# PrimeIntellect-ai/OpenDiloco

Measured on AMD Instinct MI355X. Metric: tokens_per_second, higher is better.
Workload: dtype bf16; 1 GPU; llama-150m DiLoCo, 1 worker(s), H=50, bf16, total-batch 512/worker, seq 1024 (BASELINE.json configs[1]); model=llama-150m, global_batch=512, seq_len=1024, parallelism=diloco-dp1, grad_acc=8, per_device_batch=64, params=214983680

## Files before the change

opendiloco_amd/csrc/attn.hip:

```cpp

#include "dk_common.h"
#include "../../include/diloco_kernels.h"

#include <math.h>
#include <stdlib.h>

typedef __attribute__((ext_vector_type(8))) _Float16 halfx8;

template <int DT> struct MFMA16;
template <> struct MFMA16<2> {
  using frag = shortx8;
  static __device__ __forceinline__ floatx4 mma(frag a, frag b, floatx4 c) {
    return __builtin_amdgcn_mfma_f32_16x16x32_bf16(a, b, c, 0, 0, 0);
  }
};
template <> struct MFMA16<1> {
  using frag = halfx8;
  static __device__ __forceinline__ floatx4 mma(frag a, frag b, floatx4 c) {
    return __builtin_amdgcn_mfma_f32_16x16x32_f16(a, b, c, 0, 0, 0);
  }
};

template <int DT> struct TrRead;
template <> struct TrRead<2> {
  typedef __attribute__((ext_vector_type(4))) __bf16 v4;
  static __device__ __forceinline__ void rd(const unsigned short* p, void* out) {
    v4 r = __builtin_amdgcn_ds_read_tr16_b64_v4bf16(
        (__attribute__((address_space(3))) v4*)(uintptr_t)(const void*)p);
    __builtin_memcpy(out, &r, 8);
  }
};
template <> struct TrRead<1> {
  typedef __attribute__((ext_vector_type(4))) __fp16 v4;
  static __device__ __forceinline__ void rd(const _Float16* p, void* out) {
    v4 r = __builtin_amdgcn_ds_read_tr16_b64_v4f16(
        (__attribute__((address_space(3))) v4*)(uintptr_t)(const void*)p);
    __builtin_memcpy(out, &r, 8);
  }
};
template <int DT>
__device__ __forceinline__ typename MFMA16<DT>::frag trread_bfrag(
    const typename DTraits<DT>::T* img, int row0, int col0, int ds, int lane) {
  const int rb = row0 + 8 * (lane >> 4) + ((lane & 15) >> 2);
  const int cb = col0 + 4 * (lane & 3);
  typename MFMA16<DT>::frag f;
  TrRead<DT>::rd(img + rb * ds + cb, &f);
  TrRead<DT>::rd(img + (rb + 4) * ds + cb, (char*)&f + 8);
  return f;
}

template <int DT> struct Pack4;
template <> struct Pack4<2> { using V = shortx4; };
template <> struct Pack4<1> { typedef __attribute__((ext_vector_type(4))) _Float16 V; };

#define NEG_BIG (-1e30f)

__device__ __forceinline__ float grp16_max(float x) {
#pragma unroll
  for (int off = 1; off < 16; off <<= 1) x = fmaxf(x, __shfl_xor(x, off, DK_WAVE));
  return x;
}
__device__ __forceinline__ float grp16_sum(float x) {
#pragma unroll
  for (int off = 1; off < 16; off <<= 1) x += __shfl_xor(x, off, DK_WAVE);
  return x;
}


template <int DT, int D>
__global__ __launch_bounds__(256) void attn_fwd_kernel(
    typename DTraits<DT>::T* __restrict__ o, float* __restrict__ lse,
    const typename DTraits<DT>::T* __restrict__ q,
    const typename DTraits<DT>::T* __restrict__ k,
    const typename DTraits<DT>::T* __restrict__ v,
    int B, int Hq, int Hkv, int S, float scale,
    int64_t o_sb, int64_t o_sh, int64_t o_sr,
    int64_t v_sb, int64_t v_sh, int64_t v_sr) {
  using TR = DTraits<DT>;
  using T = typename TR::T;
  using MF = MFMA16<DT>;
  using frag = typename MF::frag;
  constexpr int KT = 64;
  constexpr int KS = KT + 8;
  constexpr int DS = D + 8;
  constexpr int NKC = D / 32;
  constexpr int NDN = D / 16;
  constexpr int NNT = KT / 16;
  constexpr int LPT = (KT * D) / 8 / 256;

  extern __shared__ __attribute__((aligned(16))) char smem_raw[];
  T* K_lds = (T*)smem_raw;
  T* V_lds = K_lds + 2 * KT * DS;
  T* P_lds = V_lds + 2 * KT * DS;

  const int lane = threadIdx.x & 63;
  const int wave = threadIdx.x >> 6;
  const int lo = lane & 15;
  const int hi = lane >> 4;

  const int nQT = (S + 63) / 64;
  int bid = blockIdx.x;
  const int qt = bid % nQT;
  const int h = (bid / nQT) % Hq;
  const int b = bid / (nQT * Hq);
  const int hkv = h / (Hq / Hkv);

  const int q0 = qt * 64 + wave * 16;
  const int64_t qoff = (((int64_t)b * Hq + h) * S) * D;
  const int64_t kvoff = (((int64_t)b * Hkv + hkv) * S) * D;
  const int64_t voff = v_sb ? ((int64_t)b * v_sb + (int64_t)hkv * v_sh) : kvoff;
  const int64_t v_rs = v_sb ? v_sr : (int64_t)D;

  frag q_frag[NKC];
  {
    const int qrow = q0 + lo;
    const int qr_c = qrow < S ? qrow : S - 1;
#pragma unroll
    for (int kc = 0; kc < NKC; ++kc)
      q_frag[kc] = *(const frag*)(q + qoff + (int64_t)qr_c * D + kc * 32 + hi * 8);
  }

  float m_run[4], l_run[4];
  floatx4 o_acc[NDN];
#pragma unroll
  for (int r = 0; r < 4; ++r) { m_run[r] = NEG_BIG; l_run[r] = 0.f; }
#pragma unroll
  for (int dn = 0; dn < NDN; ++dn) o_acc[dn] = (floatx4)(0.f);

  const int kv_end = min(S, qt * 64 + 64);
  const int n_kt = (kv_end + KT - 1) / KT;

  frag kreg[LPT], vreg[LPT];
  const int st_row[2] = {(int)threadIdx.x / (D / 8), (int)(threadIdx.x + 256) / (D / 8)};
  const int st_c8[2] = {((int)threadIdx.x % (D / 8)) * 8, ((int)(threadIdx.x + 256) % (D / 8)) * 8};

  auto load_tile = [&](int kt) {
#pragma unroll
    for (int i = 0; i < LPT; ++i) {
      const int krow = kt * KT + st_row[i];
      const int kr_c = krow < S ? krow : S - 1;
      kreg[i] = *(const frag*)(k + kvoff + (int64_t)kr_c * D + st_c8[i]);
      vreg[i] = *(const frag*)(v + voff + (int64_t)kr_c * v_rs + st_c8[i]);
    }
  };
  auto write_tile = [&](int buf) {
    T* Kb = K_lds + buf * KT * DS;
    T* Vb = V_lds + buf * KT * DS;
#pragma unroll
    for (int i = 0; i < LPT; ++i) {
      *(frag*)(Kb + st_row[i] * DS + st_c8[i]) = kreg[i];
      *(frag*)(Vb + st_row[i] * DS + st_c8[i]) = vreg[i];
    }
  };

  load_tile(0);
  write_tile(0);
  __syncthreads();

  for (int kt = 0; kt < n_kt; ++kt) {
    const int kbase = kt * KT;
    const int cur = kt & 1;
    T* Kb = K_lds + cur * KT * DS;
    T* Vb = V_lds + cur * KT * DS;
    if (kt + 1 < n_kt) load_tile(kt + 1);

    floatx4 sc[NNT];
    __builtin_amdgcn_s_setprio(1);
#pragma unroll
    for (int nt = 0; nt < NNT; ++nt) {
      sc[nt] = (floatx4)(0.f);
#pragma unroll
      for (int kc = 0; kc < NKC; ++kc) {
        frag bk = *(const frag*)(Kb + (nt * 16 + lo) * DS + kc * 32 + hi * 8);
        sc[nt] = MF::mma(q_frag[kc], bk, sc[nt]);
      }
    }
    __builtin_amdgcn_s_setprio(0);

    const bool full_tile = (kbase + KT <= q0) && (kbase + KT <= S);
    float p[NNT][4];
#pragma unroll
    for (int r = 0; r < 4; ++r) {
      const int qrow = q0 + hi * 4 + r;
      float rm = NEG_BIG;
      float sv[NNT];
      if (full_tile) {
#pragma unroll
        for (int nt = 0; nt < NNT; ++nt) {
          sv[nt] = sc[nt][r] * scale;
          rm = fmaxf(rm, sv[nt]);
        }
      } else {
#pragma unroll
        for (int nt = 0; nt < NNT; ++nt) {
          const int kk = kbase + nt * 16 + lo;
          sv[nt] = (kk > qrow || kk >= S) ? NEG_BIG : sc[nt][r] * scale;
          rm = fmaxf(rm, sv[nt]);
        }
      }
      rm = grp16_max(rm);
      const float m_new = fmaxf(m_run[r], rm);
      const float alpha = __expf(m_run[r] - m_new);
      float psum = 0.f;
#pragma unroll
      for (int nt = 0; nt < NNT; ++nt) {
        p[nt][r] = sv[nt] <= NEG_BIG ? 0.f : __expf(sv[nt] - m_new);
        psum += p[nt][r];
      }
      l_run[r] = l_run[r] * alpha + grp16_sum(psum);
      m_run[r] = m_new;
#pragma unroll
      for (int dn = 0; dn < NDN; ++dn) o_acc[dn][r] *= alpha;
    }

    T* Pw = P_lds + wave * 16 * KS;
#pragma unroll
    for (int nt = 0; nt < NNT; ++nt)
#pragma unroll
      for (int r = 0; r < 4; ++r) Pw[(hi * 4 + r) * KS + nt * 16 + lo] = TR::fromF(p[nt][r]);
    frag pa[KT / 32];
#pragma unroll
    for (int c = 0; c < KT / 32; ++c)
      pa[c] = *(const frag*)(Pw + lo * KS + c * 32 + hi * 8);

    __builtin_amdgcn_s_setprio(1);
#pragma unroll
    for (int dn = 0; dn < NDN; ++dn)
#pragma unroll
      for (int c = 0; c < KT / 32; ++c) {
        frag bv = trread_bfrag<DT>(Vb, c * 32, dn * 16, DS, lane);
        o_acc[dn] = MF::mma(pa[c], bv, o_acc[dn]);
      }
    __builtin_amdgcn_s_setprio(0);

    if (kt + 1 < n_kt) write_tile((kt + 1) & 1);
    __syncthreads();
  }

#pragma unroll
  for (int r = 0; r < 4; ++r) {
    const int qrow = q0 + hi * 4 + r;
    if (qrow >= S) continue;
    const float inv_l = l_run[r] > 0.f ? 1.f / l_run[r] : 0.f;
    const int64_t obase = (int64_t)b * o_sb + (int64_t)h * o_sh + (int64_t)qrow * o_sr;
#pragma unroll
    for (int dn = 0; dn < NDN; ++dn)
      o[obase + dn * 16 + lo] = TR::fromF(o_acc[dn][r] * inv_l);
    if (lo == 0) lse[((int64_t)b * Hq + h) * S + qrow] = m_run[r] + __logf(l_run[r]);
  }
}

typedef __attribute__((ext_vector_type(16))) float floatx16;
typedef __attribute__((ext_vector_type(4))) int intx4;

template <int DT> struct MFMA32;
template <> struct MFMA32<2> {
  using frag = shortx8;
  static __device__ __forceinline__ floatx16 mma(frag a, frag b, floatx16 c) {
    return __builtin_amdgcn_mfma_f32_32x32x16_bf16(a, b, c, 0, 0, 0);
  }
};
template <> struct MFMA32<1> {
  using frag = halfx8;
  static __device__ __forceinline__ floatx16 mma(frag a, frag b, floatx16 c) {
    return __builtin_amdgcn_mfma_f32_32x32x16_f16(a, b, c, 0, 0, 0);
  }
};

template <int DT>
__device__ __forceinline__ typename MFMA32<DT>::frag trread_afrag32(
    const typename DTraits<DT>::T* img, int row0, int col0, int ds, int lane) {
  const int lam = lane & 15;
  const int rb = row0 + 8 * (lane >> 5) + (lam >> 2);
  const int cb = col0 + 16 * ((lane >> 4) & 1) + 4 * (lam & 3);
  typename MFMA32<DT>::frag f;
  TrRead<DT>::rd(img + rb * ds + cb, &f);
  TrRead<DT>::rd(img + (rb + 4) * ds + cb, (char*)&f + 8);
  return f;
}

template <int DT, int D>
__global__ __launch_bounds__(256, 4) void attn_fwd_v3_kernel(
    typename DTraits<DT>::T* __restrict__ o, float* __restrict__ lse,
    const typename DTraits<DT>::T* __restrict__ q,
    const typename DTraits<DT>::T* __restrict__ k,
    const typename DTraits<DT>::T* __restrict__ v,
    int B, int Hq, int Hkv, int S, float scale,
    int64_t o_sb, int64_t o_sh, int64_t o_sr,
    int64_t v_sb, int64_t v_sh, int64_t v_sr) {
  using TR = DTraits<DT>;
  using T = typename TR::T;
  using MF = MFMA32<DT>;
  using frag = typename MF::frag;
  constexpr int KT = 64;
  constexpr int KS = KT + 8;
  constexpr int DS = D + 8;
  constexpr int NKC = D / 16;
  constexpr int NMT = D / 32;
  constexpr int LPT = (KT * D) / 8 / 256;

  extern __shared__ __attribute__((aligned(16))) char smem_raw[];
  T* K_lds = (T*)smem_raw;
  T* V_lds = K_lds + 2 * KT * DS;

  const int lane = threadIdx.x & 63;
  const int wave = threadIdx.x >> 6;
  const int lo32 = lane & 31;
  const int hi5 = lane >> 5;

  const int nQT = (S + 127) / 128;
  int bid = blockIdx.x;
  const int qt = bid % nQT;
  const int h = (bid / nQT) % Hq;
  const int b = bid / (nQT * Hq);
  const int hkv = h / (Hq / Hkv);

  const int q0 = qt * 128 + wave * 32;
  const int qrow = q0 + lo32;
  const int64_t qoff = (((int64_t)b * Hq + h) * S) * D;
  const int64_t kvoff = (((int64_t)b * Hkv + hkv) * S) * D;
  const int64_t voff = v_sb ? ((int64_t)b * v_sb + (int64_t)hkv * v_sh) : kvoff;
  const int64_t v_rs = v_sb ? v_sr : (int64_t)D;

  frag q_frag[NKC];
  {
    const int qr_c = qrow < S ? qrow : S - 1;
#pragma unroll
    for (int kc = 0; kc < NKC; ++kc)
      q_frag[kc] = *(const frag*)(q + qoff + (int64_t)qr_c * D + kc * 16 + hi5 * 8);
  }

  float m_run = NEG_BIG, l_run = 0.f;
  floatx16 oacc[NMT];
#pragma unroll
  for (int mt = 0; mt < NMT; ++mt) oacc[mt] = (floatx16)(0.f);

  const int kv_end = min(S, qt * 128 + 128);
  const int n_kt = (kv_end + KT - 1) / KT;

  shortx8 kreg[LPT], vreg[LPT];
  const int st_row[2] = {(int)threadIdx.x / (D / 8), (int)(threadIdx.x + 256) / (D / 8)};
  const int st_c8[2] = {((int)threadIdx.x % (D / 8)) * 8, ((int)(threadIdx.x + 256) % (D / 8)) * 8};

  auto load_tile = [&](int kt) {
#pragma unroll
    for (int i = 0; i < LPT; ++i) {
      const int krow = kt * KT + st_row[i];
      const int kr_c = krow < S ? krow : S - 1;
      kreg[i] = *(const shortx8*)(k + kvoff + (int64_t)kr_c * D + st_c8[i]);
      vreg[i] = *(const shortx8*)(v + voff + (int64_t)kr_c * v_rs + st_c8[i]);
    }
  };
  auto write_tile = [&](int buf) {
    T* Kb = K_lds + buf * KT * DS;
    T* Vb = V_lds + buf * KT * DS;
#pragma unroll
    for (int i = 0; i < LPT; ++i) {
      *(shortx8*)(Kb + st_row[i] * DS + st_c8[i]) = kreg[i];
      *(shortx8*)(Vb + st_row[i] * DS + st_c8[i]) = vreg[i];
    }
  };

  load_tile(0);
  write_tile(0);
  __syncthreads();

  for (int kt = 0; kt < n_kt; ++kt) {
    const int kbase = kt * KT;
    const int cur = kt & 1;
    T* Kb = K_lds + cur * KT * DS;
    T* Vb = V_lds + cur * KT * DS;
    if (kt + 1 < n_kt) load_tile(kt + 1);

#pragma unroll
    for (int st = 0; st < 2; ++st) {
      const int sbase = kbase + st * 32;
      if (sbase >= q0 + 32) continue;
      floatx16 sc = (floatx16)(0.f);
      __builtin_amdgcn_s_setprio(1);
#pragma unroll
      for (int kc = 0; kc < NKC; ++kc) {
        frag ka = *(const frag*)(Kb + (st * 32 + lo32) * DS + kc * 16 + hi5 * 8);
        sc = MF::mma(ka, q_frag[kc], sc);
      }
      __builtin_amdgcn_s_setprio(0);

      const bool full_tile = (sbase + 32 <= q0) && (sbase + 32 <= S);
      float rm = NEG_BIG;
      if (full_tile) {
#pragma unroll
        for (int r = 0; r < 16; ++r) {
          sc[r] *= scale;
          rm = fmaxf(rm, sc[r]);
        }
      } else {
#pragma unroll
        for (int r = 0; r < 16; ++r) {
          const int key = sbase + (r & 3) + 8 * (r >> 2) + 4 * hi5;
          sc[r] = (key > qrow || key >= S) ? NEG_BIG : sc[r] * scale;
          rm = fmaxf(rm, sc[r]);
        }
      }
      rm = fmaxf(rm, __shfl_xor(rm, 32, DK_WAVE));
      const float m_new = fmaxf(m_run, rm);
      const float alpha = __expf(m_run - m_new);
      float psum = 0.f;
#pragma unroll
      for (int r = 0; r < 16; ++r) {
        sc[r] = sc[r] <= NEG_BIG ? 0.f : __expf(sc[r] - m_new);
        psum += sc[r];
      }
      psum += __shfl_xor(psum, 32, DK_WAVE);
      l_run = l_run * alpha + psum;
      m_run = m_new;
#pragma unroll
      for (int mt = 0; mt < NMT; ++mt)
#pragma unroll
        for (int r = 0; r < 16; ++r) oacc[mt][r] *= alpha;

      auto bits = [](T t) -> unsigned {
        unsigned short u;
        __builtin_memcpy(&u, &t, 2);
        return (unsigned)u;
      };
      frag pfrag[2];
#pragma unroll
      for (int c = 0; c < 2; ++c) {
        const int base = c * 8;
        unsigned w0 = bits(TR::fromF(sc[base + 0])) | (bits(TR::fromF(sc[base + 1])) << 16);
        unsigned w1 = bits(TR::fromF(sc[base + 2])) | (bits(TR::fromF(sc[base + 3])) << 16);
        unsigned w2 = bits(TR::fromF(sc[base + 4])) | (bits(TR::fromF(sc[base + 5])) << 16);
        unsigned w3 = bits(TR::fromF(sc[base + 6])) | (bits(TR::fromF(sc[base + 7])) << 16);
        auto s0 = __builtin_amdgcn_permlane32_swap((int)w0, (int)w2, false, false);
        auto s1 = __builtin_amdgcn_permlane32_swap((int)w1, (int)w3, false, false);
        intx4 pw;
        pw[0] = s0[0];
        pw[1] = s1[0];
        pw[2] = s0[1];
        pw[3] = s1[1];
        pfrag[c] = *(frag*)&pw;
      }

      __builtin_amdgcn_s_setprio(1);
#pragma unroll
      for (int mt = 0; mt < NMT; ++mt)
#pragma unroll
        for (int c = 0; c < 2; ++c) {
          frag va = trread_afrag32<DT>(Vb, st * 32 + c * 16, mt * 32, DS,
                                       (int)(threadIdx.x & 63));
          oacc[mt] = MF::mma(va, pfrag[c], oacc[mt]);
        }
      __builtin_amdgcn_s_setprio(0);
    }

    if (kt + 1 < n_kt) write_tile((kt + 1) & 1);
    __syncthreads();
  }

  if (qrow < S) {
    const float inv_l = l_run > 0.f ? 1.f / l_run : 0.f;
    const int64_t obase = (int64_t)b * o_sb + (int64_t)h * o_sh + (int64_t)qrow * o_sr;
#pragma unroll
    for (int mt = 0; mt < NMT; ++mt)
#pragma unroll
      for (int r = 0; r < 16; ++r) {
        const int d = mt * 32 + (r & 3) + 8 * (r >> 2) + 4 * hi5;
        o[obase + d] = TR::fromF(oacc[mt][r] * inv_l);
      }
    if (hi5 == 0) lse[((int64_t)b * Hq + h) * S + qrow] = m_run + __logf(l_run);
  }
}

template <int DT>
__global__ void attn_bwd_pre_kernel(float* __restrict__ delta,
                                    const typename DTraits<DT>::T* __restrict__ do_,
                                    const typename DTraits<DT>::T* __restrict__ o,
                                    int64_t rows, int H, int S, int D,
                                    int64_t g_sb, int64_t g_sh, int64_t g_sr) {
  using TR = DTraits<DT>;
  using T = typename TR::T;
  const int lane = threadIdx.x & 63;
  const int wave = threadIdx.x >> 6;
  const int lo = lane & 15, hi = lane >> 4;
  const int64_t w0 = (int64_t)blockIdx.x * 4 + wave;
  const int64_t stride = (int64_t)gridDim.x * 4;
  const int quads = D / 4;
  const int64_t groups = (rows + 3) / 4;
  for (int64_t g = w0; g < groups; g += stride) {
    const int64_t r = g * 4 + hi;
    const int64_t rc = r < rows ? r : rows - 1;
    const int sp = (int)(rc % S);
    const int hh = (int)((rc / S) % H);
    const int64_t b = rc / ((int64_t)S * H);
    const int64_t base = b * g_sb + hh * g_sh + sp * g_sr;
    float s = 0.f;
    for (int q4 = lo; q4 < quads; q4 += 16) {
      shortx4 dv = *(const shortx4*)(do_ + base + q4 * 4);
      shortx4 ov = *(const shortx4*)(o + base + q4 * 4);
      float df[4], of[4];
      packed_to_f32<DT, 4>(&dv, df);
      packed_to_f32<DT, 4>(&ov, of);
#pragma unroll
      for (int j = 0; j < 4; ++j) s += df[j] * of[j];
    }
#pragma unroll
    for (int off = 1; off < 16; off <<= 1) s += __shfl_xor(s, off, DK_WAVE);
    if (lo == 0 && r < rows) delta[r] = s;
  }
}

template <int DT, int D>
__global__ __launch_bounds__(512) void attn_bwd_dkdv_kernel(
    typename DTraits<DT>::T* __restrict__ dk_out,
    typename DTraits<DT>::T* __restrict__ dv_out,
    const typename DTraits<DT>::T* __restrict__ do_,
    const typename DTraits<DT>::T* __restrict__ q,
    const typename DTraits<DT>::T* __restrict__ k,
    const typename DTraits<DT>::T* __restrict__ v,
    const float* __restrict__ lse, const float* __restrict__ delta,
    int B, int Hq, int Hkv, int S, float scale,
    int64_t g_sb, int64_t g_sh, int64_t g_sr,
    int64_t v_sb, int64_t v_sh, int64_t v_sr,
    int64_t dv_sb, int64_t dv_sh, int64_t dv_sr) {
  using TR = DTraits<DT>;
  using T = typename TR::T;
  using MF = MFMA16<DT>;
  using frag = typename MF::frag;
  constexpr int QT = 32;
  constexpr int QTT = 64;
  constexpr int QS = QT + 8;
  constexpr int DS = D + 8;
  constexpr int NKC = D / 32;
  constexpr int NDN = D / 16;

  extern __shared__ __attribute__((aligned(16))) char smem_raw[];
  T* Q_lds = (T*)smem_raw;
  T* dO_lds = Q_lds + 2 * QTT * DS;
  T* PT_lds = dO_lds + 2 * QTT * DS;
  T* DS_lds = PT_lds + 8 * 16 * QS;
  float* lse_lds = (float*)(DS_lds + 8 * 16 * QS);
  float* dl_lds = lse_lds + 2 * QTT;

  const int lane = threadIdx.x & 63;
  const int wave = threadIdx.x >> 6;
  const int lo = lane & 15;
  const int hi = lane >> 4;

  const int nKT = (S + 127) / 128;
  int bid = blockIdx.x;
  const int kt = bid % nKT;
  const int h = (bid / nKT) % Hq;
  const int b = bid / (nKT * Hq);
  const int hkv = h / (Hq / Hkv);

  const int k0 = kt * 128 + wave * 16;
  const int64_t qoff = (((int64_t)b * Hq + h) * S) * D;
  const int64_t kvoff = (((int64_t)b * Hkv + hkv) * S) * D;
  const int64_t lseoff = ((int64_t)b * Hq + h) * S;
  const int64_t voff = v_sb ? ((int64_t)b * v_sb + (int64_t)hkv * v_sh) : kvoff;
  const int64_t v_rs = v_sb ? v_sr : (int64_t)D;

  frag k_frag[NKC], v_frag[NKC];
  {
    const int krow = k0 + lo;
    const int kr_c = krow < S ? krow : S - 1;
#pragma unroll
    for (int kc = 0; kc < NKC; ++kc) {
      k_frag[kc] = *(const frag*)(k + kvoff + (int64_t)kr_c * D + kc * 32 + hi * 8);
      v_frag[kc] = *(const frag*)(v + voff + (int64_t)kr_c * v_rs + kc * 32 + hi * 8);
    }
  }

  floatx4 dv_acc[NDN], dk_acc[NDN];
#pragma unroll
  for (int dn = 0; dn < NDN; ++dn) { dv_acc[dn] = (floatx4)(0.f); dk_acc[dn] = (floatx4)(0.f); }

  const int qstart = (kt * 128) / QTT;
  const int nQT2 = (S + QTT - 1) / QTT;

  const int st_t = (int)threadIdx.x;
  const bool st_on = st_t < (QTT * D) / 8;
  const int st_row = st_t / (D / 8);
  const int st_c8 = (st_t % (D / 8)) * 8;
  frag qreg, dreg;
  float lse_reg = 0.f, dl_reg = 0.f;

  const int64_t gbase = (int64_t)b * g_sb + (int64_t)h * g_sh;
  auto load_qtile = [&](int qt) {
    const int qrow = qt * QTT + st_row;
    const int qr_c = qrow < S ? qrow : S - 1;
    if (st_on) {
      qreg = *(const frag*)(q + qoff + (int64_t)qr_c * D + st_c8);
      dreg = *(const frag*)(do_ + gbase + (int64_t)qr_c * g_sr + st_c8);
    }
    if (st_t < QTT) {
      const int rr = qt * QTT + st_t;
      const int rr_c = rr < S ? rr : S - 1;
      lse_reg = lse[lseoff + rr_c];
      dl_reg = delta[lseoff + rr_c];
    }
  };
  auto write_qtile = [&](int buf) {
    if (st_on) {
      *(frag*)(Q_lds + buf * QTT * DS + st_row * DS + st_c8) = qreg;
      *(frag*)(dO_lds + buf * QTT * DS + st_row * DS + st_c8) = dreg;
    }
    if (st_t < QTT) {
      lse_lds[buf * QTT + st_t] = lse_reg;
      dl_lds[buf * QTT + st_t] = dl_reg;
    }
  };

  load_qtile(qstart);
  write_qtile(0);
  __syncthreads();

  for (int qt = qstart; qt < nQT2; ++qt) {
    const int cur = (qt - qstart) & 1;
    T* Q64 = Q_lds + cur * QTT * DS;
    T* dO64 = dO_lds + cur * QTT * DS;
    const float* lse64 = lse_lds + cur * QTT;
    const float* dl64 = dl_lds + cur * QTT;
    if (qt + 1 < nQT2) load_qtile(qt + 1);

#pragma unroll
    for (int hf = 0; hf < 2; ++hf) {
    const int qbase = qt * QTT + hf * QT;
    T* Qb = Q64 + hf * QT * DS;
    T* dOb = dO64 + hf * QT * DS;
    const float* lse_b = lse64 + hf * QT;
    const float* dl_b = dl64 + hf * QT;
    if (qbase + QT > k0) {
    float pt[2][4], dst[2][4];
    __builtin_amdgcn_s_setprio(1);
    const int krow = k0 + lo;
#pragma unroll
    for (int nt = 0; nt < 2; ++nt) {
      floatx4 st = (floatx4)(0.f);
      floatx4 dpt = (floatx4)(0.f);
#pragma unroll
      for (int kc = 0; kc < NKC; ++kc) {
        frag qa = *(const frag*)(Qb + (nt * 16 + lo) * DS + kc * 32 + hi * 8);
        st = MF::mma(qa, k_frag[kc], st);
        frag doa = *(const frag*)(dOb + (nt * 16 + lo) * DS + kc * 32 + hi * 8);
        dpt = MF::mma(doa, v_frag[kc], dpt);
      }
      const floatx4 lse4 = *(const floatx4*)(lse_b + nt * 16 + hi * 4);
      const floatx4 dl4 = *(const floatx4*)(dl_b + nt * 16 + hi * 4);
#pragma unroll
      for (int r = 0; r < 4; ++r) {
        const int qrow = qbase + nt * 16 + hi * 4 + r;
        float pv = 0.f;
        if (krow <= qrow && krow < S && qrow < S)
          pv = __expf(st[r] * scale - lse4[r]);
        pt[nt][r] = pv;
        dst[nt][r] = pv * (dpt[r] - dl4[r]) * scale;
      }
    }

    T* Pw = PT_lds + wave * 16 * QS;
    using P4 = typename Pack4<DT>::V;
#pragma unroll
    for (int nt = 0; nt < 2; ++nt) {
      P4 pk;
#pragma unroll
      for (int r = 0; r < 4; ++r) ((T*)&pk)[r] = TR::fromF(pt[nt][r]);
      *(P4*)(Pw + lo * QS + nt * 16 + hi * 4) = pk;
    }
    frag pa = *(const frag*)(Pw + lo * QS + hi * 8);
#pragma unroll
    for (int dn = 0; dn < NDN; ++dn) {
      frag bd = trread_bfrag<DT>(dOb, 0, dn * 16, DS, lane);
      dv_acc[dn] = MF::mma(pa, bd, dv_acc[dn]);
    }

    T* Dw = DS_lds + wave * 16 * QS;
#pragma unroll
    for (int nt = 0; nt < 2; ++nt) {
      P4 dk4;
#pragma unroll
      for (int r = 0; r < 4; ++r) ((T*)&dk4)[r] = TR::fromF(dst[nt][r]);
      *(P4*)(Dw + lo * QS + nt * 16 + hi * 4) = dk4;
    }
    frag da = *(const frag*)(Dw + lo * QS + hi * 8);
#pragma unroll
    for (int dn = 0; dn < NDN; ++dn) {
      frag bq = trread_bfrag<DT>(Qb, 0, dn * 16, DS, lane);
      dk_acc[dn] = MF::mma(da, bq, dk_acc[dn]);
    }
    __builtin_amdgcn_s_setprio(0);
    }
    }

    if (qt + 1 < nQT2) write_qtile(cur ^ 1);
    __syncthreads();
  }

  const int64_t dvoff = dv_sb ? ((int64_t)b * dv_sb + (int64_t)h * dv_sh) : qoff;
  const int64_t dv_rs = dv_sb ? dv_sr : (int64_t)D;
#pragma unroll
  for (int r = 0; r < 4; ++r) {
    const int krow = k0 + hi * 4 + r;
    if (krow >= S) continue;
#pragma unroll
    for (int dn = 0; dn < NDN; ++dn) {
      dk_out[qoff + (int64_t)krow * D + dn * 16 + lo] = TR::fromF(dk_acc[dn][r]);
      dv_out[dvoff + (int64_t)krow * dv_rs + dn * 16 + lo] = TR::fromF(dv_acc[dn][r]);
    }
  }
}

template <int DT, int D>
__global__ __launch_bounds__(512) void attn_bwd_dq_kernel(
    typename DTraits<DT>::T* __restrict__ dq_out,
    const typename DTraits<DT>::T* __restrict__ do_,
    const typename DTraits<DT>::T* __restrict__ q,
    const typename DTraits<DT>::T* __restrict__ k,
    const typename DTraits<DT>::T* __restrict__ v,
    const float* __restrict__ lse, const float* __restrict__ delta,
    int B, int Hq, int Hkv, int S, float scale,
    int64_t g_sb, int64_t g_sh, int64_t g_sr,
    int64_t v_sb, int64_t v_sh, int64_t v_sr) {
  using TR = DTraits<DT>;
  using T = typename TR::T;
  using MF = MFMA16<DT>;
  using frag = typename MF::frag;
  constexpr int KT = 64;
  constexpr int KS = KT + 8;
  constexpr int DS = D + 8;
  constexpr int NKC = D / 32;
  constexpr int NDN = D / 16;

  extern __shared__ __attribute__((aligned(16))) char smem_raw[];
  T* K_lds = (T*)smem_raw;
  T* V_lds = K_lds + 3 * KT * DS;
  T* S_lds = V_lds + 3 * KT * DS;

  const int lane = threadIdx.x & 63;
  const int wave = threadIdx.x >> 6;
  const int lo = lane & 15;
  const int hi = lane >> 4;

  const int nQT = (S + 127) / 128;
  int bid = blockIdx.x;
  const int qt = bid % nQT;
  const int h = (bid / nQT) % Hq;
  const int b = bid / (nQT * Hq);
  const int hkv = h / (Hq / Hkv);

  const int q0 = qt * 128 + wave * 16;
  const int64_t qoff = (((int64_t)b * Hq + h) * S) * D;
  const int64_t kvoff = (((int64_t)b * Hkv + hkv) * S) * D;
  const int64_t lseoff = ((int64_t)b * Hq + h) * S;
  const int64_t voff = v_sb ? ((int64_t)b * v_sb + (int64_t)hkv * v_sh) : kvoff;
  const int64_t v_rs = v_sb ? v_sr : (int64_t)D;

  frag q_frag[NKC], do_frag[NKC];
  float lse_q, dl_q;
  const int qrow_l = q0 + lo;
  {
    const int qr_c = qrow_l < S ? qrow_l : S - 1;
    const int64_t gbase = (int64_t)b * g_sb + (int64_t)h * g_sh;
#pragma unroll
    for (int kc = 0; kc < NKC; ++kc) {
      q_frag[kc] = *(const frag*)(q + qoff + (int64_t)qr_c * D + kc * 32 + hi * 8);
      do_frag[kc] = *(const frag*)(do_ + gbase + (int64_t)qr_c * g_sr + kc * 32 + hi * 8);
    }
    lse_q = lse[lseoff + qr_c];
    dl_q = delta[lseoff + qr_c];
  }

  floatx4 dq_acc[NDN];
#pragma unroll
  for (int dn = 0; dn < NDN; ++dn) dq_acc[dn] = (floatx4)(0.f);

  const int kv_end = min(S, qt * 128 + 128);
  const int n_kt = (kv_end + KT - 1) / KT;

  const int st_t = (int)threadIdx.x;
  const bool st_on = st_t < (KT * D) / 8;
  const int st_row = st_t / (D / 8);
  const int st_c8 = (st_t % (D / 8)) * 8;
  frag kregA, vregA, kregB, vregB;

  auto load_ktile = [&](int kt, frag& kr, frag& vr) {
    if (st_on) {
      const int krow = kt * KT + st_row;
      const int kr_c = krow < S ? krow : S - 1;
      kr = *(const frag*)(k + kvoff + (int64_t)kr_c * D + st_c8);
      vr = *(const frag*)(v + voff + (int64_t)kr_c * v_rs + st_c8);
    }
  };
  auto write_ktile = [&](int buf, const frag& kr, const frag& vr) {
    if (st_on) {
      *(frag*)(K_lds + buf * KT * DS + st_row * DS + st_c8) = kr;
      *(frag*)(V_lds + buf * KT * DS + st_row * DS + st_c8) = vr;
    }
  };

  load_ktile(0, kregA, vregA);
  write_ktile(0, kregA, vregA);
  if (1 < n_kt) load_ktile(1, kregB, vregB);
  __syncthreads();

  for (int kt = 0; kt < n_kt; ++kt) {
    const int kbase = kt * KT;
    const int cur = kt % 3;
    T* Kb = K_lds + cur * KT * DS;
    T* Vb = V_lds + cur * KT * DS;
    if (kt + 2 < n_kt) {
      if ((kt + 2) & 1) load_ktile(kt + 2, kregB, vregB);
      else load_ktile(kt + 2, kregA, vregA);
    }

    if (kbase < q0 + 16) {
    float ds[4][4];
    __builtin_amdgcn_s_setprio(1);
#pragma unroll
    for (int nt = 0; nt < 4; ++nt) {
      floatx4 st = (floatx4)(0.f), dpt = (floatx4)(0.f);
#pragma unroll
      for (int kc = 0; kc < NKC; ++kc) {
        frag ka = *(const frag*)(Kb + (nt * 16 + lo) * DS + kc * 32 + hi * 8);
        st = MF::mma(ka, q_frag[kc], st);
        frag va = *(const frag*)(Vb + (nt * 16 + lo) * DS + kc * 32 + hi * 8);
        dpt = MF::mma(va, do_frag[kc], dpt);
      }
#pragma unroll
      for (int r = 0; r < 4; ++r) {
        const int kcol = kbase + nt * 16 + hi * 4 + r;
        float pv = 0.f;
        if (kcol <= qrow_l && kcol < S && qrow_l < S)
          pv = __expf(st[r] * scale - lse_q);
        ds[nt][r] = pv * (dpt[r] - dl_q) * scale;
      }
    }

    T* Sw = S_lds + wave * 16 * KS;
    using P4 = typename Pack4<DT>::V;
#pragma unroll
    for (int nt = 0; nt < 4; ++nt) {
      P4 s4;
#pragma unroll
      for (int r = 0; r < 4; ++r) ((T*)&s4)[r] = TR::fromF(ds[nt][r]);
      *(P4*)(Sw + lo * KS + nt * 16 + hi * 4) = s4;
    }
    frag da[2];
#pragma unroll
    for (int c = 0; c < 2; ++c) da[c] = *(const frag*)(Sw + lo * KS + c * 32 + hi * 8);
#pragma unroll
    for (int dn = 0; dn < NDN; ++dn)
#pragma unroll
      for (int c = 0; c < 2; ++c) {
        frag bk = trread_bfrag<DT>(Kb, c * 32, dn * 16, DS, lane);
        dq_acc[dn] = MF::mma(da[c], bk, dq_acc[dn]);
      }
    __builtin_amdgcn_s_setprio(0);
    }

    if (kt + 1 < n_kt) {
      if ((kt + 1) & 1) write_ktile((kt + 1) % 3, kregB, vregB);
      else write_ktile((kt + 1) % 3, kregA, vregA);
    }
    __syncthreads();
  }

#pragma unroll
  for (int r = 0; r < 4; ++r) {
    const int qrow = q0 + hi * 4 + r;
    if (qrow >= S) continue;
#pragma unroll
    for (int dn = 0; dn < NDN; ++dn)
      dq_out[qoff + (int64_t)qrow * D + dn * 16 + lo] = TR::fromF(dq_acc[dn][r]);
  }
}


template <int DT, int D>
__global__ __launch_bounds__(256) void attn_bwd_dkdv_v3_kernel(
    typename DTraits<DT>::T* __restrict__ dk_out,
    typename DTraits<DT>::T* __restrict__ dv_out,
    const typename DTraits<DT>::T* __restrict__ do_,
    const typename DTraits<DT>::T* __restrict__ q,
    const typename DTraits<DT>::T* __restrict__ k,
    const typename DTraits<DT>::T* __restrict__ v,
    const float* __restrict__ lse, const float* __restrict__ delta,
    int B, int Hq, int Hkv, int S, float scale,
    int64_t g_sb, int64_t g_sh, int64_t g_sr) {
  using TR = DTraits<DT>;
  using T = typename TR::T;
  using MF = MFMA32<DT>;
  using frag = typename MF::frag;
  constexpr int QT = 32;
  constexpr int QS = QT + 8;
  constexpr int DS = D + 8;
  constexpr int NKC = D / 16;
  constexpr int NMT = D / 32;

  extern __shared__ __attribute__((aligned(16))) char smem_raw[];
  T* Q_lds = (T*)smem_raw;
  T* dO_lds = Q_lds + 2 * QT * DS;
  T* PT_lds = dO_lds + 2 * QT * DS;
  T* DST_lds = PT_lds + 4 * 32 * QS;
  float* lse_lds = (float*)(DST_lds + 4 * 32 * QS);
  float* dl_lds = lse_lds + 2 * QT;

  const int lane = threadIdx.x & 63;
  const int wave = threadIdx.x >> 6;
  const int lo32 = lane & 31;
  const int hi5 = lane >> 5;

  const int nKT = (S + 127) / 128;
  int bid = blockIdx.x;
  const int kt = bid % nKT;
  const int h = (bid / nKT) % Hq;
  const int b = bid / (nKT * Hq);
  const int hkv = h / (Hq / Hkv);

  const int k0 = kt * 128 + wave * 32;
  const int64_t qoff = (((int64_t)b * Hq + h) * S) * D;
  const int64_t kvoff = (((int64_t)b * Hkv + hkv) * S) * D;
  const int64_t lseoff = ((int64_t)b * Hq + h) * S;

  const int kr_c0 = (k0 + lo32) < S ? (k0 + lo32) : S - 1;
  const T* kbase_p = k + kvoff + (int64_t)kr_c0 * D + hi5 * 8;
  const T* vbase_p = v + kvoff + (int64_t)kr_c0 * D + hi5 * 8;

  floatx16 dv_acc[NMT], dk_acc[NMT];
#pragma unroll
  for (int mt = 0; mt < NMT; ++mt) { dv_acc[mt] = (floatx16)(0.f); dk_acc[mt] = (floatx16)(0.f); }

  const int qstart = (kt * 128) / QT;
  const int nQT2 = (S + QT - 1) / QT;

  const int st_t = (int)threadIdx.x;
  const bool st_on = st_t < (QT * D) / 8;
  const int st_row = st_t / (D / 8);
  const int st_c8 = (st_t % (D / 8)) * 8;
  shortx8 qreg, dreg;
  float lse_reg = 0.f, dl_reg = 0.f;
  const int64_t gbase = (int64_t)b * g_sb + (int64_t)h * g_sh;

  auto load_qtile = [&](int qt2) {
    const int qrow = qt2 * QT + st_row;
    const int qr_c = qrow < S ? qrow : S - 1;
    if (st_on) {
      qreg = *(const shortx8*)(q + qoff + (int64_t)qr_c * D + st_c8);
      dreg = *(const shortx8*)(do_ + gbase + (int64_t)qr_c * g_sr + st_c8);
    }
    if (st_t < QT) {
      const int rr = qt2 * QT + st_t;
      const int rr_c = rr < S ? rr : S - 1;
      lse_reg = lse[lseoff + rr_c];
      dl_reg = delta[lseoff + rr_c];
    }
  };
  auto write_qtile = [&](int buf) {
    if (st_on) {
      *(shortx8*)(Q_lds + buf * QT * DS + st_row * DS + st_c8) = qreg;
      *(shortx8*)(dO_lds + buf * QT * DS + st_row * DS + st_c8) = dreg;
    }
    if (st_t < QT) {
      lse_lds[buf * QT + st_t] = lse_reg;
      dl_lds[buf * QT + st_t] = dl_reg;
    }
  };

  load_qtile(qstart);
  write_qtile(0);
  __syncthreads();

  for (int qt2 = qstart; qt2 < nQT2; ++qt2) {
    const int qbase = qt2 * QT;
    const int cur = (qt2 - qstart) & 1;
    T* Qb = Q_lds + cur * QT * DS;
    T* dOb = dO_lds + cur * QT * DS;
    const float* lse_b = lse_lds + cur * QT;
    const float* dl_b = dl_lds + cur * QT;
    if (qt2 + 1 < nQT2) load_qtile(qt2 + 1);

    floatx16 st = (floatx16)(0.f), dpt = (floatx16)(0.f);
    __builtin_amdgcn_s_setprio(1);
#pragma unroll
    for (int kc = 0; kc < NKC; ++kc) {
      frag ka = *(const frag*)(kbase_p + kc * 16);
      frag bq = *(const frag*)(Qb + lo32 * DS + kc * 16 + hi5 * 8);
      st = MF::mma(ka, bq, st);
      frag va = *(const frag*)(vbase_p + kc * 16);
      frag bd = *(const frag*)(dOb + lo32 * DS + kc * 16 + hi5 * 8);
      dpt = MF::mma(va, bd, dpt);
    }
    __builtin_amdgcn_s_setprio(0);

    const int qcol = qbase + lo32;
    const float lse_q = lse_b[lo32];
    const float dl_q = dl_b[lo32];
    const bool full = (qbase >= k0 + 32) && (qbase + QT <= S);
    float pt[16], dst[16];
#pragma unroll
    for (int r = 0; r < 16; ++r) {
      float pv;
      if (full) {
        pv = __expf(st[r] * scale - lse_q);
      } else {
        const int krow = k0 + (r & 3) + 8 * (r >> 2) + 4 * hi5;
        pv = 0.f;
        if (krow <= qcol && krow < S && qcol < S)
          pv = __expf(st[r] * scale - lse_q);
      }
      pt[r] = pv;
      dst[r] = pv * (dpt[r] - dl_q) * scale;
    }

    T* Pw = PT_lds + wave * 32 * QS;
#pragma unroll
    for (int r = 0; r < 16; ++r)
      Pw[((r & 3) + 8 * (r >> 2) + 4 * hi5) * QS + lo32] = TR::fromF(pt[r]);
    frag pa[2];
#pragma unroll
    for (int c = 0; c < 2; ++c)
      pa[c] = *(const frag*)(Pw + lo32 * QS + c * 16 + hi5 * 8);
    __builtin_amdgcn_s_setprio(1);
#pragma unroll
    for (int mt = 0; mt < NMT; ++mt)
#pragma unroll
      for (int c = 0; c < 2; ++c) {
        frag bd = trread_afrag32<DT>(dOb, c * 16, mt * 32, DS, lane);
        dv_acc[mt] = MF::mma(pa[c], bd, dv_acc[mt]);
      }
    __builtin_amdgcn_s_setprio(0);

    T* Dw = DST_lds + wave * 32 * QS;
#pragma unroll
    for (int r = 0; r < 16; ++r)
      Dw[((r & 3) + 8 * (r >> 2) + 4 * hi5) * QS + lo32] = TR::fromF(dst[r]);
    frag da[2];
#pragma unroll
    for (int c = 0; c < 2; ++c)
      da[c] = *(const frag*)(Dw + lo32 * QS + c * 16 + hi5 * 8);
    __builtin_amdgcn_s_setprio(1);
#pragma unroll
    for (int mt = 0; mt < NMT; ++mt)
#pragma unroll
      for (int c = 0; c < 2; ++c) {
        frag bq = trread_afrag32<DT>(Qb, c * 16, mt * 32, DS, lane);
        dk_acc[mt] = MF::mma(da[c], bq, dk_acc[mt]);
      }
    __builtin_amdgcn_s_setprio(0);

    if (qt2 + 1 < nQT2) write_qtile(cur ^ 1);
    __syncthreads();
  }

#pragma unroll
  for (int r = 0; r < 16; ++r) {
    const int krow = k0 + (r & 3) + 8 * (r >> 2) + 4 * hi5;
    if (krow >= S) continue;
#pragma unroll
    for (int mt = 0; mt < NMT; ++mt) {
      dk_out[qoff + (int64_t)krow * D + mt * 32 + lo32] = TR::fromF(dk_acc[mt][r]);
      dv_out[qoff + (int64_t)krow * D + mt * 32 + lo32] = TR::fromF(dv_acc[mt][r]);
    }
  }
}

template <int DT, int D, int WANT_DK>
__global__ __launch_bounds__(256) void attn_bwd_split32_kernel(
    typename DTraits<DT>::T* __restrict__ out,
    const typename DTraits<DT>::T* __restrict__ do_,
    const typename DTraits<DT>::T* __restrict__ q,
    const typename DTraits<DT>::T* __restrict__ k,
    const typename DTraits<DT>::T* __restrict__ v,
    const float* __restrict__ lse, const float* __restrict__ delta,
    int B, int Hq, int Hkv, int S, float scale,
    int64_t g_sb, int64_t g_sh, int64_t g_sr,
    int64_t v_sb, int64_t v_sh, int64_t v_sr,
    int64_t o_sb, int64_t o_sh, int64_t o_sr) {
  using TR = DTraits<DT>;
  using T = typename TR::T;
  using MF = MFMA32<DT>;
  using frag = typename MF::frag;
  using P4 = typename Pack4<DT>::V;
  constexpr int QT = 32;
  constexpr int QS = QT + 8;
  constexpr int DS = D + 8;
  constexpr int NKC = D / 16;
  constexpr int NMT = D / 32;

  extern __shared__ __attribute__((aligned(16))) char smem_raw[];
  T* Q_lds = (T*)smem_raw;
  T* dO_lds = Q_lds + 2 * QT * DS;
  T* PT_lds = dO_lds + 2 * QT * DS;
  float* lse_lds = (float*)(PT_lds + 4 * 32 * QS);
  float* dl_lds = lse_lds + 2 * QT;

  const int lane = threadIdx.x & 63;
  const int wave = threadIdx.x >> 6;
  const int lo32 = lane & 31;
  const int hi5 = lane >> 5;

  const int nKT = (S + 127) / 128;
  int bid = blockIdx.x;
  const int kt = bid % nKT;
  const int h = (bid / nKT) % Hq;
  const int b = bid / (nKT * Hq);
  const int hkv = h / (Hq / Hkv);

  const int k0 = kt * 128 + wave * 32;
  const int64_t qoff = (((int64_t)b * Hq + h) * S) * D;
  const int64_t kvoff = (((int64_t)b * Hkv + hkv) * S) * D;
  const int64_t lseoff = ((int64_t)b * Hq + h) * S;
  const int64_t voff = v_sb ? ((int64_t)b * v_sb + (int64_t)hkv * v_sh) : kvoff;
  const int64_t v_rs = v_sb ? v_sr : (int64_t)D;

  const int kr_c0 = (k0 + lo32) < S ? (k0 + lo32) : S - 1;
  const T* kbase_p = k + kvoff + (int64_t)kr_c0 * D + hi5 * 8;
  const T* vbase_p = v + voff + (int64_t)kr_c0 * v_rs + hi5 * 8;

  floatx16 acc[NMT];
#pragma unroll
  for (int mt = 0; mt < NMT; ++mt) acc[mt] = (floatx16)(0.f);

  const int qstart = (kt * 128) / QT;
  const int nQT2 = (S + QT - 1) / QT;

  const int st_t = (int)threadIdx.x;
  const bool st_on = st_t < (QT * D) / 8;
  const int st_row = st_t / (D / 8);
  const int st_c8 = (st_t % (D / 8)) * 8;
  shortx8 qreg, dreg;
  float lse_reg = 0.f, dl_reg = 0.f;
  const int64_t gbase = (int64_t)b * g_sb + (int64_t)h * g_sh;

  auto load_qtile = [&](int qt2) {
    const int qrow = qt2 * QT + st_row;
    const int qr_c = qrow < S ? qrow : S - 1;
    if (st_on) {
      qreg = *(const shortx8*)(q + qoff + (int64_t)qr_c * D + st_c8);
      dreg = *(const shortx8*)(do_ + gbase + (int64_t)qr_c * g_sr + st_c8);
    }
    if (st_t < QT) {
      const int rr = qt2 * QT + st_t;
      const int rr_c = rr < S ? rr : S - 1;
      lse_reg = lse[lseoff + rr_c];
      if (WANT_DK) dl_reg = delta[lseoff + rr_c];
    }
  };
  auto write_qtile = [&](int buf) {
    if (st_on) {
      *(shortx8*)(Q_lds + buf * QT * DS + st_row * DS + st_c8) = qreg;
      *(shortx8*)(dO_lds + buf * QT * DS + st_row * DS + st_c8) = dreg;
    }
    if (st_t < QT) {
      lse_lds[buf * QT + st_t] = lse_reg;
      if (WANT_DK) dl_lds[buf * QT + st_t] = dl_reg;
    }
  };

  load_qtile(qstart);
  write_qtile(0);
  __syncthreads();

  for (int qt2 = qstart; qt2 < nQT2; ++qt2) {
    const int qbase = qt2 * QT;
    const int cur = (qt2 - qstart) & 1;
    T* Qb = Q_lds + cur * QT * DS;
    T* dOb = dO_lds + cur * QT * DS;
    const float* lse_b = lse_lds + cur * QT;
    const float* dl_b = dl_lds + cur * QT;
    if (qt2 + 1 < nQT2) load_qtile(qt2 + 1);

    floatx16 st = (floatx16)(0.f), dpt = (floatx16)(0.f);
    __builtin_amdgcn_s_setprio(1);
#pragma unroll
    for (int kc = 0; kc < NKC; ++kc) {
      frag qa = *(const frag*)(Qb + lo32 * DS + kc * 16 + hi5 * 8);
      frag kb = *(const frag*)(kbase_p + kc * 16);
      st = MF::mma(qa, kb, st);
      if (WANT_DK) {
        frag doa = *(const frag*)(dOb + lo32 * DS + kc * 16 + hi5 * 8);
        frag vb = *(const frag*)(vbase_p + kc * 16);
        dpt = MF::mma(doa, vb, dpt);
      }
    }
    __builtin_amdgcn_s_setprio(0);

    const int krow = k0 + lo32;
    const bool full = (qbase >= k0 + 32) && (qbase + QT <= S);
    T* Pw = PT_lds + wave * 32 * QS;
#pragma unroll
    for (int g = 0; g < 4; ++g) {
      const int qloc = 8 * g + 4 * hi5;
      const floatx4 lse4 = *(const floatx4*)(lse_b + qloc);
      floatx4 dl4;
      if (WANT_DK) dl4 = *(const floatx4*)(dl_b + qloc);
      P4 pk;
#pragma unroll
      for (int r = 0; r < 4; ++r) {
        const int i = g * 4 + r;
        float pv;
        if (full) {
          pv = __expf(st[i] * scale - lse4[r]);
        } else {
          const int qrow = qbase + qloc + r;
          pv = 0.f;
          if (krow <= qrow && krow < S && qrow < S)
            pv = __expf(st[i] * scale - lse4[r]);
        }
        if (WANT_DK) pv = pv * (dpt[i] - dl4[r]) * scale;
        ((T*)&pk)[r] = TR::fromF(pv);
      }
      *(P4*)(Pw + lo32 * QS + qloc) = pk;
    }

    frag pa[2];
#pragma unroll
    for (int c = 0; c < 2; ++c)
      pa[c] = *(const frag*)(Pw + lo32 * QS + c * 16 + hi5 * 8);
    __builtin_amdgcn_s_setprio(1);
#pragma unroll
    for (int mt = 0; mt < NMT; ++mt)
#pragma unroll
      for (int c = 0; c < 2; ++c) {
        frag bb = trread_afrag32<DT>(WANT_DK ? Qb : dOb, c * 16, mt * 32, DS, lane);
        acc[mt] = MF::mma(pa[c], bb, acc[mt]);
      }
    __builtin_amdgcn_s_setprio(0);

    if (qt2 + 1 < nQT2) write_qtile(cur ^ 1);
    __syncthreads();
  }

  const int64_t obase = o_sb ? ((int64_t)b * o_sb + (int64_t)h * o_sh) : qoff;
  const int64_t o_rs = o_sb ? o_sr : (int64_t)D;
#pragma unroll
  for (int r = 0; r < 16; ++r) {
    const int kr = k0 + (r & 3) + 8 * (r >> 2) + 4 * hi5;
    if (kr >= S) continue;
#pragma unroll
    for (int mt = 0; mt < NMT; ++mt)
      out[obase + (int64_t)kr * o_rs + mt * 32 + lo32] = TR::fromF(acc[mt][r]);
  }
}

template <int DT, int D>
__global__ __launch_bounds__(256) void attn_bwd_dq_v3_kernel(
    typename DTraits<DT>::T* __restrict__ dq_out,
    const typename DTraits<DT>::T* __restrict__ do_,
    const typename DTraits<DT>::T* __restrict__ q,
    const typename DTraits<DT>::T* __restrict__ k,
    const typename DTraits<DT>::T* __restrict__ v,
    const float* __restrict__ lse, const float* __restrict__ delta,
    int B, int Hq, int Hkv, int S, float scale,
    int64_t g_sb, int64_t g_sh, int64_t g_sr) {
  using TR = DTraits<DT>;
  using T = typename TR::T;
  using MF = MFMA32<DT>;
  using frag = typename MF::frag;
  constexpr int KT = 32;
  constexpr int KS = KT + 8;
  constexpr int DS = D + 8;
  constexpr int NKC = D / 16;
  constexpr int NMT = D / 32;

  extern __shared__ __attribute__((aligned(16))) char smem_raw[];
  T* K_lds = (T*)smem_raw;
  T* V_lds = K_lds + 2 * KT * DS;
  T* S_lds = V_lds + 2 * KT * DS;

  const int lane = threadIdx.x & 63;
  const int wave = threadIdx.x >> 6;
  const int lo32 = lane & 31;
  const int hi5 = lane >> 5;

  const int nQT = (S + 127) / 128;
  int bid = blockIdx.x;
  const int qt = bid % nQT;
  const int h = (bid / nQT) % Hq;
  const int b = bid / (nQT * Hq);
  const int hkv = h / (Hq / Hkv);

  const int q0 = qt * 128 + wave * 32;
  const int64_t qoff = (((int64_t)b * Hq + h) * S) * D;
  const int64_t kvoff = (((int64_t)b * Hkv + hkv) * S) * D;
  const int64_t lseoff = ((int64_t)b * Hq + h) * S;

  frag q_frag[NKC], do_frag[NKC];
  float lse_r[16], dl_r[16];
  {
    const int qrow = q0 + lo32;
    const int qr_c = qrow < S ? qrow : S - 1;
    const int64_t gb = (int64_t)b * g_sb + (int64_t)h * g_sh;
#pragma unroll
    for (int kc = 0; kc < NKC; ++kc) {
      q_frag[kc] = *(const frag*)(q + qoff + (int64_t)qr_c * D + kc * 16 + hi5 * 8);
      do_frag[kc] = *(const frag*)(do_ + gb + (int64_t)qr_c * g_sr + kc * 16 + hi5 * 8);
    }
#pragma unroll
    for (int r = 0; r < 16; ++r) {
      const int rr = q0 + (r & 3) + 8 * (r >> 2) + 4 * hi5;
      const int rr_c = rr < S ? rr : S - 1;
      lse_r[r] = lse[lseoff + rr_c];
      dl_r[r] = delta[lseoff + rr_c];
    }
  }

  floatx16 dq_acc[NMT];
#pragma unroll
  for (int mt = 0; mt < NMT; ++mt) dq_acc[mt] = (floatx16)(0.f);

  const int kv_end = min(S, qt * 128 + 128);
  const int n_kt = (kv_end + KT - 1) / KT;

  const int st_t = (int)threadIdx.x;
  const bool st_on = st_t < (KT * D) / 8;
  const int st_row = st_t / (D / 8);
  const int st_c8 = (st_t % (D / 8)) * 8;
  shortx8 kreg, vreg;

  auto load_ktile = [&](int kt2) {
    if (st_on) {
      const int krow = kt2 * KT + st_row;
      const int kr_c = krow < S ? krow : S - 1;
      kreg = *(const shortx8*)(k + kvoff + (int64_t)kr_c * D + st_c8);
      vreg = *(const shortx8*)(v + kvoff + (int64_t)kr_c * D + st_c8);
    }
  };
  auto write_ktile = [&](int buf) {
    if (st_on) {
      *(shortx8*)(K_lds + buf * KT * DS + st_row * DS + st_c8) = kreg;
      *(shortx8*)(V_lds + buf * KT * DS + st_row * DS + st_c8) = vreg;
    }
  };

  load_ktile(0);
  write_ktile(0);
  __syncthreads();

  for (int kt2 = 0; kt2 < n_kt; ++kt2) {
    const int kbase = kt2 * KT;
    const int cur = kt2 & 1;
    T* Kb = K_lds + cur * KT * DS;
    T* Vb = V_lds + cur * KT * DS;
    if (kt2 + 1 < n_kt) load_ktile(kt2 + 1);

    floatx16 st = (floatx16)(0.f), dpt = (floatx16)(0.f);
    __builtin_amdgcn_s_setprio(1);
#pragma unroll
    for (int kc = 0; kc < NKC; ++kc) {
      frag bk = *(const frag*)(Kb + lo32 * DS + kc * 16 + hi5 * 8);
      st = MF::mma(q_frag[kc], bk, st);
      frag bv = *(const frag*)(Vb + lo32 * DS + kc * 16 + hi5 * 8);
      dpt = MF::mma(do_frag[kc], bv, dpt);
    }
    __builtin_amdgcn_s_setprio(0);

    const int kcol = kbase + lo32;
    const bool full = (kbase + KT <= q0) && (kbase + KT <= S) && (q0 + 32 <= S);
    float ds[16];
#pragma unroll
    for (int r = 0; r < 16; ++r) {
      float pv;
      if (full) {
        pv = __expf(st[r] * scale - lse_r[r]);
      } else {
        const int qrow = q0 + (r & 3) + 8 * (r >> 2) + 4 * hi5;
        pv = 0.f;
        if (kcol <= qrow && kcol < S && qrow < S)
          pv = __expf(st[r] * scale - lse_r[r]);
      }
      ds[r] = pv * (dpt[r] - dl_r[r]) * scale;
    }

    T* Sw = S_lds + wave * 32 * KS;
#pragma unroll
    for (int r = 0; r < 16; ++r)
      Sw[((r & 3) + 8 * (r >> 2) + 4 * hi5) * KS + lo32] = TR::fromF(ds[r]);
    frag da[2];
#pragma unroll
    for (int c = 0; c < 2; ++c)
      da[c] = *(const frag*)(Sw + lo32 * KS + c * 16 + hi5 * 8);
    __builtin_amdgcn_s_setprio(1);
#pragma unroll
    for (int mt = 0; mt < NMT; ++mt)
#pragma unroll
      for (int c = 0; c < 2; ++c) {
        frag bk = trread_afrag32<DT>(Kb, c * 16, mt * 32, DS, lane);
        dq_acc[mt] = MF::mma(da[c], bk, dq_acc[mt]);
      }
    __builtin_amdgcn_s_setprio(0);

    if (kt2 + 1 < n_kt) write_ktile(cur ^ 1);
    __syncthreads();
  }

#pragma unroll
  for (int r = 0; r < 16; ++r) {
    const int qrow = q0 + (r & 3) + 8 * (r >> 2) + 4 * hi5;
    if (qrow >= S) continue;
#pragma unroll
    for (int mt = 0; mt < NMT; ++mt)
      dq_out[qoff + (int64_t)qrow * D + mt * 32 + lo32] = TR::fromF(dq_acc[mt][r]);
  }
}


static bool use_attn_v2() {
  static int cached = -1;
  if (cached < 0) {
    const char* e = getenv("DK_ATTN_V2");
    cached = (e && e[0] == '1') ? 1 : 0;
  }
  return cached == 1;
}

static bool use_bwd_split32() {
  static int v = -1;
  if (v < 0) {
    const char* e = getenv("DK_ATTN_BWD_SPLIT32");
    v = (e && e[0] == '1') ? 1 : 0;
  }
  return v != 0;
}

static bool use_bwd_v3() {
  static int cached = -1;
  if (cached < 0) {
    const char* e = getenv("DK_ATTN_BWD_V3");
    cached = (e && e[0] == '1') ? 1 : 0;
  }
  return cached == 1;
}

template <int DT, int D>
static int launch_attn_fwd(void* o, float* lse, const void* q, const void* k,
                           const void* v, int64_t B, int64_t Hq, int64_t Hkv,
                           int64_t S, float scale, int64_t o_sb, int64_t o_sh,
                           int64_t o_sr, int64_t v_sb, int64_t v_sh, int64_t v_sr,
                           dkStream stream) {
  using T = typename DTraits<DT>::T;
  constexpr int KT = 64, KS = KT + 8, DS = D + 8;
  if (!use_attn_v2()) {
    const int nQT = (int)((S + 127) / 128);
    const int grid = (int)(B * Hq * nQT);
    const size_t lds = sizeof(T) * (2 * KT * DS + 2 * KT * DS);
    hipLaunchKernelGGL((attn_fwd_v3_kernel<DT, D>), dim3(grid), dim3(256), lds,
                       (hipStream_t)stream, (T*)o, lse, (const T*)q, (const T*)k,
                       (const T*)v, (int)B, (int)Hq, (int)Hkv, (int)S, scale,
                       o_sb, o_sh, o_sr, v_sb, v_sh, v_sr);
    DK_CHECK_LAUNCH();
    return 0;
  }
  const int nQT = (int)((S + 63) / 64);
  const int grid = (int)(B * Hq * nQT);
  const size_t lds = sizeof(T) * (2 * KT * DS + 2 * KT * DS + 4 * 16 * KS);
  hipLaunchKernelGGL((attn_fwd_kernel<DT, D>), dim3(grid), dim3(256), lds,
                     (hipStream_t)stream, (T*)o, lse, (const T*)q, (const T*)k,
                     (const T*)v, (int)B, (int)Hq, (int)Hkv, (int)S, scale,
                     o_sb, o_sh, o_sr, v_sb, v_sh, v_sr);
  DK_CHECK_LAUNCH();
  return 0;
}

extern "C" int dk_attn_fwd(void* o, float* lse, const void* q, const void* k,
                           const void* v, int64_t B, int64_t Hq, int64_t Hkv,
                           int64_t S, int64_t D, float scale,
                           int64_t o_sb, int64_t o_sh, int64_t o_sr,
                           int64_t v_sb, int64_t v_sh, int64_t v_sr, int dtype,
                           dkStream stream) {
  if (dtype != 1 && dtype != 2) return (int)hipErrorInvalidValue;
  if (o_sb == 0) { o_sb = Hq * S * D; o_sh = S * D; o_sr = D; }
  if (D == 64) {
    if (dtype == 2) return launch_attn_fwd<2, 64>(o, lse, q, k, v, B, Hq, Hkv, S, scale, o_sb, o_sh, o_sr, v_sb, v_sh, v_sr, stream);
    return launch_attn_fwd<1, 64>(o, lse, q, k, v, B, Hq, Hkv, S, scale, o_sb, o_sh, o_sr, v_sb, v_sh, v_sr, stream);
  } else if (D == 32) {
    if (dtype == 2) return launch_attn_fwd<2, 32>(o, lse, q, k, v, B, Hq, Hkv, S, scale, o_sb, o_sh, o_sr, v_sb, v_sh, v_sr, stream);
    return launch_attn_fwd<1, 32>(o, lse, q, k, v, B, Hq, Hkv, S, scale, o_sb, o_sh, o_sr, v_sb, v_sh, v_sr, stream);
  }
  return (int)hipErrorInvalidValue;
}

extern "C" int dk_attn_bwd_preprocess(float* delta, const void* do_, const void* o,
                                      int64_t B, int64_t H, int64_t S, int64_t D,
                                      int64_t g_sb, int64_t g_sh, int64_t g_sr,
                                      int dtype, dkStream stream) {
  const int64_t rows = B * H * S;
  if (g_sb == 0) { g_sb = H * S * D; g_sh = S * D; g_sr = D; }
  int64_t g = (rows + 3) / 4;
  int grid = (int)(g > 2048 ? 2048 : (g < 1 ? 1 : g));
  DK_DISPATCH_DT(dtype, {
    if constexpr (kDT != 0) {
      using T = typename DTraits<kDT>::T;
      hipLaunchKernelGGL((attn_bwd_pre_kernel<kDT>), dim3(grid), dim3(256), 0,
                         (hipStream_t)stream, delta, (const T*)do_, (const T*)o,
                         rows, (int)H, (int)S, (int)D, g_sb, g_sh, g_sr);
    } else {
      return (int)hipErrorInvalidValue;
    }
  });
  DK_CHECK_LAUNCH();
  return 0;
}

template <int DT, int D>
static int launch_attn_bwd_dkdv(void* dk_o, void* dv_o, const void* do_, const void* q,
                                const void* k, const void* v, const float* lse,
                                const float* delta, int64_t B, int64_t Hq, int64_t Hkv,
                                int64_t S, float scale, int64_t g_sb, int64_t g_sh,
                                int64_t g_sr, int64_t v_sb, int64_t v_sh, int64_t v_sr,
                                int64_t dv_sb, int64_t dv_sh, int64_t dv_sr,
                                dkStream stream) {
  using T = typename DTraits<DT>::T;
  constexpr int QT = 32, QS = QT + 8, DS = D + 8;
  if (use_bwd_split32()) {
    const int nKTs = (int)((S + 127) / 128);
    const int grids = (int)(B * Hq * nKTs);
    const size_t ldss = sizeof(T) * (4 * QT * DS + 4 * 32 * QS) + sizeof(float) * 4 * QT;
    hipLaunchKernelGGL((attn_bwd_split32_kernel<DT, D, 0>), dim3(grids), dim3(256), ldss,
                       (hipStream_t)stream, (T*)dv_o, (const T*)do_, (const T*)q,
                       (const T*)k, (const T*)v, lse, delta, (int)B, (int)Hq,
                       (int)Hkv, (int)S, scale, g_sb, g_sh, g_sr, v_sb, v_sh, v_sr,
                       dv_sb, dv_sh, dv_sr);
    DK_CHECK_LAUNCH();
    hipLaunchKernelGGL((attn_bwd_split32_kernel<DT, D, 1>), dim3(grids), dim3(256), ldss,
                       (hipStream_t)stream, (T*)dk_o, (const T*)do_, (const T*)q,
                       (const T*)k, (const T*)v, lse, delta, (int)B, (int)Hq,
                       (int)Hkv, (int)S, scale, g_sb, g_sh, g_sr, v_sb, v_sh, v_sr,
                       0, 0, 0);
    DK_CHECK_LAUNCH();
    return 0;
  }
  if (use_bwd_v3() && v_sb == 0 && dv_sb == 0) {
    const int nKT3 = (int)((S + 127) / 128);
    const int grid3 = (int)(B * Hq * nKT3);
    const size_t lds3 = sizeof(T) * (4 * QT * DS + 2 * 4 * 32 * QS)
                        + sizeof(float) * 4 * QT;
    hipLaunchKernelGGL((attn_bwd_dkdv_v3_kernel<DT, D>), dim3(grid3), dim3(256), lds3,
                       (hipStream_t)stream, (T*)dk_o, (T*)dv_o, (const T*)do_,
                       (const T*)q, (const T*)k, (const T*)v, lse, delta,
                       (int)B, (int)Hq, (int)Hkv, (int)S, scale, g_sb, g_sh, g_sr);
    DK_CHECK_LAUNCH();
    return 0;
  }
  const int nKT = (int)((S + 127) / 128);
  const int grid = (int)(B * Hq * nKT);
  constexpr int QTT = 64;
  const size_t lds = sizeof(T) * (4 * QTT * DS + 2 * 8 * 16 * QS) + sizeof(float) * 4 * QTT;
  hipLaunchKernelGGL((attn_bwd_dkdv_kernel<DT, D>), dim3(grid), dim3(512), lds,
                     (hipStream_t)stream, (T*)dk_o, (T*)dv_o, (const T*)do_,
                     (const T*)q, (const T*)k, (const T*)v, lse, delta,
                     (int)B, (int)Hq, (int)Hkv, (int)S, scale, g_sb, g_sh, g_sr,
                     v_sb, v_sh, v_sr, dv_sb, dv_sh, dv_sr);
  DK_CHECK_LAUNCH();
  return 0;
}

extern "C" int dk_attn_bwd_dkdv(void* dk_o, void* dv_o, const void* do_, const void* q,
                                const void* k, const void* v, const float* lse,
                                const float* delta, int64_t B, int64_t Hq, int64_t Hkv,
                                int64_t S, int64_t D, float scale,
                                int64_t g_sb, int64_t g_sh, int64_t g_sr,
                                int64_t v_sb, int64_t v_sh, int64_t v_sr,
                                int64_t dv_sb, int64_t dv_sh, int64_t dv_sr, int dtype,
                                dkStream stream) {
  if (dtype != 1 && dtype != 2) return (int)hipErrorInvalidValue;
  if (g_sb == 0) { g_sb = Hq * S * D; g_sh = S * D; g_sr = D; }
  if (D == 64) {
    if (dtype == 2) return launch_attn_bwd_dkdv<2, 64>(dk_o, dv_o, do_, q, k, v, lse, delta, B, Hq, Hkv, S, scale, g_sb, g_sh, g_sr, v_sb, v_sh, v_sr, dv_sb, dv_sh, dv_sr, stream);
    return launch_attn_bwd_dkdv<1, 64>(dk_o, dv_o, do_, q, k, v, lse, delta, B, Hq, Hkv, S, scale, g_sb, g_sh, g_sr, v_sb, v_sh, v_sr, dv_sb, dv_sh, dv_sr, stream);
  } else if (D == 32) {
    if (dtype == 2) return launch_attn_bwd_dkdv<2, 32>(dk_o, dv_o, do_, q, k, v, lse, delta, B, Hq, Hkv, S, scale, g_sb, g_sh, g_sr, v_sb, v_sh, v_sr, dv_sb, dv_sh, dv_sr, stream);
    return launch_attn_bwd_dkdv<1, 32>(dk_o, dv_o, do_, q, k, v, lse, delta, B, Hq, Hkv, S, scale, g_sb, g_sh, g_sr, v_sb, v_sh, v_sr, dv_sb, dv_sh, dv_sr, stream);
  }
  return (int)hipErrorInvalidValue;
}

template <int DT, int D>
static int launch_attn_bwd_dq(void* dq_o, const void* do_, const void* q, const void* k,
                              const void* v, const float* lse, const float* delta,
                              int64_t B, int64_t Hq, int64_t Hkv, int64_t S,
                              float scale, int64_t g_sb, int64_t g_sh, int64_t g_sr,
                              int64_t v_sb, int64_t v_sh, int64_t v_sr,
                              dkStream stream) {
  using T = typename DTraits<DT>::T;
  constexpr int KT = 32, KS = KT + 8, DS = D + 8;
  constexpr int KT2 = 64, KS2 = KT2 + 8;
  if (use_bwd_v3() && v_sb == 0) {
    const int nQT3 = (int)((S + 127) / 128);
    const int grid3 = (int)(B * Hq * nQT3);
    const size_t lds3 = sizeof(T) * (4 * KT * DS + 4 * 32 * KS);
    hipLaunchKernelGGL((attn_bwd_dq_v3_kernel<DT, D>), dim3(grid3), dim3(256), lds3,
                       (hipStream_t)stream, (T*)dq_o, (const T*)do_, (const T*)q,
                       (const T*)k, (const T*)v, lse, delta, (int)B, (int)Hq,
                       (int)Hkv, (int)S, scale, g_sb, g_sh, g_sr);
    DK_CHECK_LAUNCH();
    return 0;
  }
  const int nQT = (int)((S + 127) / 128);
  const int grid = (int)(B * Hq * nQT);
  const size_t lds = sizeof(T) * (6 * KT2 * DS + 8 * 16 * KS2);
  hipLaunchKernelGGL((attn_bwd_dq_kernel<DT, D>), dim3(grid), dim3(512), lds,
                     (hipStream_t)stream, (T*)dq_o, (const T*)do_, (const T*)q,
                     (const T*)k, (const T*)v, lse, delta, (int)B, (int)Hq,
                     (int)Hkv, (int)S, scale, g_sb, g_sh, g_sr, v_sb, v_sh, v_sr);
  DK_CHECK_LAUNCH();
  return 0;
}

extern "C" int dk_attn_bwd_dq(void* dq_o, const void* do_, const void* q, const void* k,
                              const void* v, const float* lse, const float* delta,
                              int64_t B, int64_t Hq, int64_t Hkv, int64_t S, int64_t D,
                              float scale, int64_t g_sb, int64_t g_sh, int64_t g_sr,
                              int64_t v_sb, int64_t v_sh, int64_t v_sr,
                              int dtype, dkStream stream) {
  if (dtype != 1 && dtype != 2) return (int)hipErrorInvalidValue;
  if (g_sb == 0) { g_sb = Hq * S * D; g_sh = S * D; g_sr = D; }
  if (D == 64) {
    if (dtype == 2) return launch_attn_bwd_dq<2, 64>(dq_o, do_, q, k, v, lse, delta, B, Hq, Hkv, S, scale, g_sb, g_sh, g_sr, v_sb, v_sh, v_sr, stream);
    return launch_attn_bwd_dq<1, 64>(dq_o, do_, q, k, v, lse, delta, B, Hq, Hkv, S, scale, g_sb, g_sh, g_sr, v_sb, v_sh, v_sr, stream);
  } else if (D == 32) {
    if (dtype == 2) return launch_attn_bwd_dq<2, 32>(dq_o, do_, q, k, v, lse, delta, B, Hq, Hkv, S, scale, g_sb, g_sh, g_sr, v_sb, v_sh, v_sr, stream);
    return launch_attn_bwd_dq<1, 32>(dq_o, do_, q, k, v, lse, delta, B, Hq, Hkv, S, scale, g_sb, g_sh, g_sr, v_sb, v_sh, v_sr, stream);
  }
  return (int)hipErrorInvalidValue;
}

__global__ void probe_mfma_kernel(float* __restrict__ out,
                                  const unsigned short* __restrict__ a,
                                  const unsigned short* __restrict__ b) {
  const int lane = threadIdx.x & 63;
  const int lo = lane & 15, hi = lane >> 4;
  shortx8 af, bf;
#pragma unroll
  for (int j = 0; j < 8; ++j) {
    ((unsigned short*)&af)[j] = a[lo * 32 + hi * 8 + j];
    ((unsigned short*)&bf)[j] = b[(hi * 8 + j) * 16 + lo];
  }
  floatx4 c = (floatx4)(0.f);
  c = __builtin_amdgcn_mfma_f32_16x16x32_bf16(af, bf, c, 0, 0, 0);
#pragma unroll
  for (int r = 0; r < 4; ++r) out[(hi * 4 + r) * 16 + lo] = c[r];
}

extern "C" int dk_probe_mfma_16x16x32_bf16(float* out_d, const void* a16x32,
                                           const void* b32x16, dkStream stream) {
  hipLaunchKernelGGL(probe_mfma_kernel, dim3(1), dim3(64), 0, (hipStream_t)stream,
                     out_d, (const unsigned short*)a16x32, (const unsigned short*)b32x16);
  DK_CHECK_LAUNCH();
  return 0;
}

__global__ void probe_mfma_alt_kernel(float* __restrict__ out,
                                      const unsigned short* __restrict__ a,
                                      const unsigned short* __restrict__ b) {
  const int lane = threadIdx.x & 63;
  const int lo = lane & 15, hi = lane >> 4;
  shortx8 af, bf;
#pragma unroll
  for (int j = 0; j < 8; ++j) {
    ((unsigned short*)&af)[j] = a[lo * 32 + (hi + 4 * j)];
    ((unsigned short*)&bf)[j] = b[(hi + 4 * j) * 16 + lo];
  }
  floatx4 c = (floatx4)(0.f);
  c = __builtin_amdgcn_mfma_f32_16x16x32_bf16(af, bf, c, 0, 0, 0);
#pragma unroll
  for (int r = 0; r < 4; ++r) out[(hi * 4 + r) * 16 + lo] = c[r];
}

extern "C" int dk_probe_mfma_16x16x32_bf16_alt(float* out_d, const void* a16x32,
                                               const void* b32x16, dkStream stream) {
  hipLaunchKernelGGL(probe_mfma_alt_kernel, dim3(1), dim3(64), 0, (hipStream_t)stream,
                     out_d, (const unsigned short*)a16x32, (const unsigned short*)b32x16);
  DK_CHECK_LAUNCH();
  return 0;
}

typedef __attribute__((ext_vector_type(16))) float floatx16;
__global__ void probe_mfma32_kernel(float* __restrict__ out,
                                    const unsigned short* __restrict__ a,
                                    const unsigned short* __restrict__ b) {
  const int lane = threadIdx.x & 63;
  const int lo = lane & 31, hi = lane >> 5;
  shortx8 af, bf;
#pragma unroll
  for (int j = 0; j < 8; ++j) {
    ((unsigned short*)&af)[j] = a[lo * 16 + hi * 8 + j];
    ((unsigned short*)&bf)[j] = b[(hi * 8 + j) * 32 + lo];
  }
  floatx16 c = (floatx16)(0.f);
  c = __builtin_amdgcn_mfma_f32_32x32x16_bf16(af, bf, c, 0, 0, 0);
#pragma unroll
  for (int r = 0; r < 16; ++r)
    out[((r & 3) + 8 * (r >> 2) + 4 * hi) * 32 + lo] = c[r];
}

extern "C" int dk_probe_mfma_32x32x16_bf16(float* out_d, const void* a32x16,
                                           const void* b16x32, dkStream stream) {
  hipLaunchKernelGGL(probe_mfma32_kernel, dim3(1), dim3(64), 0, (hipStream_t)stream,
                     out_d, (const unsigned short*)a32x16, (const unsigned short*)b16x32);
  DK_CHECK_LAUNCH();
  return 0;
}

__global__ void probe_permlane_kernel(int* __restrict__ out) {
  const int lane = threadIdx.x & 63;
  int a = lane, b = 100 + lane;
  auto r = __builtin_amdgcn_permlane32_swap(a, b, false, false);
  out[lane] = r[0];
  out[64 + lane] = r[1];
}

extern "C" int dk_probe_permlane32(int* out_d, dkStream stream) {
  hipLaunchKernelGGL(probe_permlane_kernel, dim3(1), dim3(64), 0, (hipStream_t)stream, out_d);
  DK_CHECK_LAUNCH();
  return 0;
}
```

Measured before the change: 611,200 tokens/s.

## Rewrite attention backward dq and dkdv kernels with 32x32 MFMA register fragments

Both attention backward kernels (dq and dk/dv) are rebuilt around 32x32x16 MFMA tiles with 256-thread blocks. The score and dS fragments are packed in registers via permlane32_swap instead of round-tripping through LDS scratch. The softmax exponent becomes exp2 with LSE and delta folded in early, and the experimental v3/split32 backward paths and their env switches are removed. The intent is to cut LDS traffic and instruction count and raise occupancy. The cost is higher register pressure, and the new alignment check on the dv output can reject strides the old path accepted.

```diff
diff --git a/opendiloco_amd/csrc/attn.hip b/opendiloco_amd/csrc/attn.hip
--- a/opendiloco_amd/csrc/attn.hip
+++ b/opendiloco_amd/csrc/attn.hip
@@ -279,6 +279,35 @@
   return f;
 }
 
+template <int DT> struct Pack2;
+template <> struct Pack2<2> { typedef __attribute__((ext_vector_type(2))) __bf16 V; };
+template <> struct Pack2<1> { typedef __attribute__((ext_vector_type(2))) _Float16 V; };
+template <int DT>
+__device__ __forceinline__ unsigned cvt_pk2(float a, float b) {
+  typedef __attribute__((ext_vector_type(2))) float f2;
+  typename Pack2<DT>::V r = __builtin_convertvector((f2){a, b}, typename Pack2<DT>::V);
+  unsigned u;
+  __builtin_memcpy(&u, &r, 4);
+  return u;
+}
+
+template <int DT>
+__device__ __forceinline__ typename MFMA32<DT>::frag pack_frag32(const floatx16& x, int c) {
+  const int base = c * 8;
+  const unsigned w0 = cvt_pk2<DT>(x[base + 0], x[base + 1]);
+  const unsigned w1 = cvt_pk2<DT>(x[base + 2], x[base + 3]);
+  const unsigned w2 = cvt_pk2<DT>(x[base + 4], x[base + 5]);
+  const unsigned w3 = cvt_pk2<DT>(x[base + 6], x[base + 7]);
+  auto s0 = __builtin_amdgcn_permlane32_swap((int)w0, (int)w2, false, false);
+  auto s1 = __builtin_amdgcn_permlane32_swap((int)w1, (int)w3, false, false);
+  intx4 pw;
+  pw[0] = s0[0];
+  pw[1] = s1[0];
+  pw[2] = s0[1];
+  pw[3] = s1[1];
+  return *(typename MFMA32<DT>::frag*)&pw;
+}
+
 template <int DT, int D>
 __global__ __launch_bounds__(256, 4) void attn_fwd_v3_kernel(
     typename DTraits<DT>::T* __restrict__ o, float* __restrict__ lse,
@@ -418,28 +447,9 @@
 #pragma unroll
         for (int r = 0; r < 16; ++r) oacc[mt][r] *= alpha;
 
-      auto bits = [](T t) -> unsigned {
-        unsigned short u;
-        __builtin_memcpy(&u, &t, 2);
-        return (unsigned)u;
-      };
       frag pfrag[2];
 #pragma unroll
-      for (int c = 0; c < 2; ++c) {
-        const int base = c * 8;
-        unsigned w0 = bits(TR::fromF(sc[base + 0])) | (bits(TR::fromF(sc[base + 1])) << 16);
-        unsigned w1 = bits(TR::fromF(sc[base + 2])) | (bits(TR::fromF(sc[base + 3])) << 16);
-        unsigned w2 = bits(TR::fromF(sc[base + 4])) | (bits(TR::fromF(sc[base + 5])) << 16);
-        unsigned w3 = bits(TR::fromF(sc[base + 6])) | (bits(TR::fromF(sc[base + 7])) << 16);
-        auto s0 = __builtin_amdgcn_permlane32_swap((int)w0, (int)w2, false, false);
-        auto s1 = __builtin_amdgcn_permlane32_swap((int)w1, (int)w3, false, false);
-        intx4 pw;
-        pw[0] = s0[0];
-        pw[1] = s1[0];
-        pw[2] = s0[1];
-        pw[3] = s1[1];
-        pfrag[c] = *(frag*)&pw;
-      }
+      for (int c = 0; c < 2; ++c) pfrag[c] = pack_frag32<DT>(sc, c);
 
       __builtin_amdgcn_s_setprio(1);
 #pragma unroll
@@ -509,8 +519,176 @@
   }
 }
 
+
+__device__ __forceinline__ float exp2_fast(float x) { return __builtin_amdgcn_exp2f(x); }
+
+template <int DT>
+__device__ __forceinline__ void store4(typename DTraits<DT>::T* dst, const floatx16& x,
+                                       int g, float mul) {
+  using P4 = typename Pack4<DT>::V;
+  P4 pk;
+#pragma unroll
+  for (int i = 0; i < 4; ++i) ((typename DTraits<DT>::T*)&pk)[i] = DTraits<DT>::fromF(x[4 * g + i] * mul);
+  *(P4*)dst = pk;
+}
+
 template <int DT, int D>
-__global__ __launch_bounds__(512) void attn_bwd_dkdv_kernel(
+__global__ __launch_bounds__(256, 3) void attn_bwd_dq_kernel(
+    typename DTraits<DT>::T* __restrict__ dq_out,
+    const typename DTraits<DT>::T* __restrict__ do_,
+    const typename DTraits<DT>::T* __restrict__ q,
+    const typename DTraits<DT>::T* __restrict__ k,
+    const typename DTraits<DT>::T* __restrict__ v,
+    const float* __restrict__ lse, const float* __restrict__ delta,
+    int B, int Hq, int Hkv, int S, float scale,
+    int64_t g_sb, int64_t g_sh, int64_t g_sr,
+    int64_t v_sb, int64_t v_sh, int64_t v_sr) {
+  using TR = DTraits<DT>;
+  using T = typename TR::T;
+  using MF = MFMA32<DT>;
+  using frag = typename MF::frag;
+  constexpr int KT = 64;
+  constexpr int DS = D + 8;
+  constexpr int NKC = D / 16;
+  constexpr int NMT = D / 32;
+  constexpr int LPT = (KT * D) / 8 / 256;
+
+  extern __shared__ __attribute__((aligned(16))) char smem_raw[];
+  T* K_lds = (T*)smem_raw;
+  T* V_lds = K_lds + 2 * KT * DS;
+
+  const int lane = threadIdx.x & 63;
+  const int wave = threadIdx.x >> 6;
+  const int lo32 = lane & 31;
+  const int hi5 = lane >> 5;
+
+  const int nQT = (S + 127) / 128;
+  int bid = blockIdx.x;
+  const int qt = bid % nQT;
+  const int h = (bid / nQT) % Hq;
+  const int b = bid / (nQT * Hq);
+  const int hkv = h / (Hq / Hkv);
+
+  const int q0 = qt * 128 + wave * 32;
+  const int qrow = q0 + lo32;
+  const int64_t qoff = (((int64_t)b * Hq + h) * S) * D;
+  const int64_t kvoff = (((int64_t)b * Hkv + hkv) * S) * D;
+  const int64_t lseoff = ((int64_t)b * Hq + h) * S;
+  const int64_t voff = v_sb ? ((int64_t)b * v_sb + (int64_t)hkv * v_sh) : kvoff;
+  const int64_t v_rs = v_sb ? v_sr : (int64_t)D;
+  const int64_t gbase = (int64_t)b * g_sb + (int64_t)h * g_sh;
+
+  frag q_frag[NKC], do_frag[NKC];
+  float nl2, dl_q;
+  {
+    const int qr_c = qrow < S ? qrow : S - 1;
+#pragma unroll
+    for (int kc = 0; kc < NKC; ++kc) {
+      q_frag[kc] = *(const frag*)(q + qoff + (int64_t)qr_c * D + kc * 16 + hi5 * 8);
+      do_frag[kc] = *(const frag*)(do_ + gbase + (int64_t)qr_c * g_sr + kc * 16 + hi5 * 8);
+    }
+    nl2 = -lse[lseoff + qr_c] * 1.4426950408889634f;
+    dl_q = delta[lseoff + qr_c];
+  }
+  const float c2 = scale * 1.4426950408889634f;
+
+  floatx16 dq_acc[NMT];
+#pragma unroll
+  for (int mt = 0; mt < NMT; ++mt) dq_acc[mt] = (floatx16)(0.f);
+
+  const int kv_end = min(S, qt * 128 + 128);
+  const int n_kt = (kv_end + KT - 1) / KT;
+
+  shortx8 kreg[LPT], vreg[LPT];
+  int st_row[LPT], st_c8[LPT];
+#pragma unroll
+  for (int i = 0; i < LPT; ++i) {
+    st_row[i] = (int)(threadIdx.x + 256 * i) / (D / 8);
+    st_c8[i] = ((int)(threadIdx.x + 256 * i) % (D / 8)) * 8;
+  }
+  auto load_tile = [&](int kt) {
+#pragma unroll
+    for (int i = 0; i < LPT; ++i) {
+      const int krow = kt * KT + st_row[i];
+      const int kr_c = krow < S ? krow : S - 1;
+      kreg[i] = *(const shortx8*)(k + kvoff + (int64_t)kr_c * D + st_c8[i]);
+      vreg[i] = *(const shortx8*)(v + voff + (int64_t)kr_c * v_rs + st_c8[i]);
+    }
+  };
+  auto write_tile = [&](int buf) {
+    T* Kb = K_lds + buf * KT * DS;
+    T* Vb = V_lds + buf * KT * DS;
+#pragma unroll
+    for (int i = 0; i < LPT; ++i) {
+      *(shortx8*)(Kb + st_row[i] * DS + st_c8[i]) = kreg[i];
+      *(shortx8*)(Vb + st_row[i] * DS + st_c8[i]) = vreg[i];
+    }
+  };
+
+  load_tile(0);
+  write_tile(0);
+  __syncthreads();
+
+  for (int kt = 0; kt < n_kt; ++kt) {
+    const int cur = kt & 1;
+    const T* Kb = K_lds + cur * KT * DS;
+    const T* Vb = V_lds + cur * KT * DS;
+    if (kt + 1 < n_kt) load_tile(kt + 1);
+
+#pragma unroll
+    for (int st = 0; st < 2; ++st) {
+      const int sbase = kt * KT + st * 32;
+      if (sbase >= q0 + 32) continue;
+      floatx16 sc = (floatx16)(0.f), dp = (floatx16)(0.f);
+      __builtin_amdgcn_s_setprio(1);
+#pragma unroll
+      for (int kc = 0; kc < NKC; ++kc) {
+        frag ka = *(const frag*)(Kb + (st * 32 + lo32) * DS + kc * 16 + hi5 * 8);
+        sc = MF::mma(ka, q_frag[kc], sc);
+        frag va = *(const frag*)(Vb + (st * 32 + lo32) * DS + kc * 16 + hi5 * 8);
+        dp = MF::mma(va, do_frag[kc], dp);
+      }
+      __builtin_amdgcn_s_setprio(0);
+
+#pragma unroll
+      for (int r = 0; r < 16; ++r) dp[r] = (dp[r] - dl_q) * exp2_fast(fmaf(sc[r], c2, nl2));
+      if (sbase >= q0) {
+#pragma unroll
+        for (int r = 0; r < 16; ++r) {
+          const int key = sbase + (r & 3) + 8 * (r >> 2) + 4 * hi5;
+          if (key > qrow) dp[r] = 0.f;
+        }
+      }
+      frag dsf[2];
+#pragma unroll
+      for (int c = 0; c < 2; ++c) dsf[c] = pack_frag32<DT>(dp, c);
+
+      __builtin_amdgcn_s_setprio(1);
+#pragma unroll
+      for (int mt = 0; mt < NMT; ++mt)
+#pragma unroll
+        for (int c = 0; c < 2; ++c) {
+          frag ka = trread_afrag32<DT>(Kb, st * 32 + c * 16, mt * 32, DS, lane);
+          dq_acc[mt] = MF::mma(ka, dsf[c], dq_acc[mt]);
+        }
+      __builtin_amdgcn_s_setprio(0);
+    }
+
+    if (kt + 1 < n_kt) write_tile((kt + 1) & 1);
+    __syncthreads();
+  }
+
+  if (qrow < S) {
+    T* dst = dq_out + qoff + (int64_t)qrow * D;
+#pragma unroll
+    for (int mt = 0; mt < NMT; ++mt)
+#pragma unroll
+      for (int g = 0; g < 4; ++g) store4<DT>(dst + mt * 32 + 8 * g + 4 * hi5, dq_acc[mt], g, scale);
+  }
+}
+
+template <int DT, int D>
+__global__ __launch_bounds__(256, 3) void attn_bwd_dkdv_kernel(
     typename DTraits<DT>::T* __restrict__ dk_out,
     typename DTraits<DT>::T* __restrict__ dv_out,
     const typename DTraits<DT>::T* __restrict__ do_,
@@ -524,27 +702,26 @@
     int64_t dv_sb, int64_t dv_sh, int64_t dv_sr) {
   using TR = DTraits<DT>;
   using T = typename TR::T;
-  using MF = MFMA16<DT>;
+  using MF = MFMA32<DT>;
   using frag = typename MF::frag;
   constexpr int QT = 32;
-  constexpr int QTT = 64;
-  constexpr int QS = QT + 8;
+  constexpr int QTT = 32;
   constexpr int DS = D + 8;
-  constexpr int NKC = D / 32;
-  constexpr int NDN = D / 16;
+  constexpr int NKC = D / 16;
+  constexpr int NMT = D / 32;
+  constexpr int NCH = (QTT * D) / 8;
+  constexpr int LPT = (NCH + 255) / 256;
 
   extern __shared__ __attribute__((aligned(16))) char smem_raw[];
   T* Q_lds = (T*)smem_raw;
   T* dO_lds = Q_lds + 2 * QTT * DS;
-  T* PT_lds = dO_lds + 2 * QTT * DS;
-  T* DS_lds = PT_lds + 8 * 16 * QS;
-  float* lse_lds = (float*)(DS_lds + 8 * 16 * QS);
+  float* lse_lds = (float*)(dO_lds + 2 * QTT * DS);
   float* dl_lds = lse_lds + 2 * QTT;
 
   const int lane = threadIdx.x & 63;
   const int wave = threadIdx.x >> 6;
-  const int lo = lane & 15;
-  const int hi = lane >> 4;
+  const int lo32 = lane & 31;
+  const int hi5 = lane >> 5;
 
   const int nKT = (S + 127) / 128;
   int bid = blockIdx.x;
@@ -553,57 +730,64 @@
   const int b = bid / (nKT * Hq);
   const int hkv = h / (Hq / Hkv);
 
-  const int k0 = kt * 128 + wave * 16;
+  const int k0 = kt * 128 + wave * 32;
+  const int key = k0 + lo32;
   const int64_t qoff = (((int64_t)b * Hq + h) * S) * D;
   const int64_t kvoff = (((int64_t)b * Hkv + hkv) * S) * D;
   const int64_t lseoff = ((int64_t)b * Hq + h) * S;
   const int64_t voff = v_sb ? ((int64_t)b * v_sb + (int64_t)hkv * v_sh) : kvoff;
   const int64_t v_rs = v_sb ? v_sr : (int64_t)D;
+  const int64_t gbase = (int64_t)b * g_sb + (int64_t)h * g_sh;
 
   frag k_frag[NKC], v_frag[NKC];
   {
-    const int krow = k0 + lo;
-    const int kr_c = krow < S ? krow : S - 1;
+    const int kr_c = key < S ? key : S - 1;
 #pragma unroll
     for (int kc = 0; kc < NKC; ++kc) {
-      k_frag[kc] = *(const frag*)(k + kvoff + (int64_t)kr_c * D + kc * 32 + hi * 8);
-      v_frag[kc] = *(const frag*)(v + voff + (int64_t)kr_c * v_rs + kc * 32 + hi * 8);
-    }
-  }
-
-  floatx4 dv_acc[NDN], dk_acc[NDN];
-#pragma unroll
-  for (int dn = 0; dn < NDN; ++dn) { dv_acc[dn] = (floatx4)(0.f); dk_acc[dn] = (floatx4)(0.f); }
+      k_frag[kc] = *(const frag*)(k + kvoff + (int64_t)kr_c * D + kc * 16 + hi5 * 8);
+      v_frag[kc] = *(const frag*)(v + voff + (int64_t)kr_c * v_rs + kc * 16 + hi5 * 8);
+    }
+  }
+  const float c2 = scale * 1.4426950408889634f;
+
+  floatx16 dv_acc[NMT], dk_acc[NMT];
+#pragma unroll
+  for (int mt = 0; mt < NMT; ++mt) { dv_acc[mt] = (floatx16)(0.f); dk_acc[mt] = (floatx16)(0.f); }
 
   const int qstart = (kt * 128) / QTT;
   const int nQT2 = (S + QTT - 1) / QTT;
 
+  shortx8 qreg[LPT], dreg[LPT];
+  float lse_reg = 0.f, dl_reg = 0.f;
+  int st_row[LPT], st_c8[LPT];
+#pragma unroll
+  for (int i = 0; i < LPT; ++i) {
+    st_row[i] = (int)(threadIdx.x + 256 * i) / (D / 8);
+    st_c8[i] = ((int)(threadIdx.x + 256 * i) % (D / 8)) * 8;
+  }
   const int st_t = (int)threadIdx.x;
-  const bool st_on = st_t < (QTT * D) / 8;
-  const int st_row = st_t / (D / 8);
-  const int st_c8 = (st_t % (D / 8)) * 8;
-  frag qreg, dreg;
-  float lse_reg = 0.f, dl_reg = 0.f;
-
-  const int64_t gbase = (int64_t)b * g_sb + (int64_t)h * g_sh;
   auto load_qtile = [&](int qt) {
-    const int qrow = qt * QTT + st_row;
-    const int qr_c = qrow < S ? qrow : S - 1;
-    if (st_on) {
-      qreg = *(const frag*)(q + qoff + (int64_t)qr_c * D + st_c8);
-      dreg = *(const frag*)(do_ + gbase + (int64_t)qr_c * g_sr + st_c8);
+#pragma unroll
+    for (int i = 0; i < LPT; ++i) {
+      if (NCH % 256 && (int)threadIdx.x + 256 * i >= NCH) break;
+      const int qr = qt * QTT + st_row[i];
+      const int qr_c = qr < S ? qr : S - 1;
+      qreg[i] = *(const shortx8*)(q + qoff + (int64_t)qr_c * D + st_c8[i]);
+      dreg[i] = *(const shortx8*)(do_ + gbase + (int64_t)qr_c * g_sr + st_c8[i]);
     }
     if (st_t < QTT) {
       const int rr = qt * QTT + st_t;
       const int rr_c = rr < S ? rr : S - 1;
-      lse_reg = lse[lseoff + rr_c];
-      dl_reg = delta[lseoff + rr_c];
+      lse_reg = -lse[lseoff + rr_c] / scale;
+      dl_reg = -delta[lseoff + rr_c];
     }
   };
   auto write_qtile = [&](int buf) {
-    if (st_on) {
-      *(frag*)(Q_lds + buf * QTT * DS + st_row * DS + st_c8) = qreg;
-      *(frag*)(dO_lds + buf * QTT * DS + st_row * DS + st_c8) = dreg;
+#pragma unroll
+    for (int i = 0; i < LPT; ++i) {
+      if (NCH % 256 && (int)threadIdx.x + 256 * i >= NCH) break;
+      *(shortx8*)(Q_lds + buf * QTT * DS + st_row[i] * DS + st_c8[i]) = qreg[i];
+      *(shortx8*)(dO_lds + buf * QTT * DS + st_row[i] * DS + st_c8[i]) = dreg[i];
     }
     if (st_t < QTT) {
       lse_lds[buf * QTT + st_t] = lse_reg;
@@ -617,790 +801,82 @@
 
   for (int qt = qstart; qt < nQT2; ++qt) {
     const int cur = (qt - qstart) & 1;
-    T* Q64 = Q_lds + cur * QTT * DS;
-    T* dO64 = dO_lds + cur * QTT * DS;
-    const float* lse64 = lse_lds + cur * QTT;
-    const float* dl64 = dl_lds + cur * QTT;
     if (qt + 1 < nQT2) load_qtile(qt + 1);
 
 #pragma unroll
-    for (int hf = 0; hf < 2; ++hf) {
-    const int qbase = qt * QTT + hf * QT;
-    T* Qb = Q64 + hf * QT * DS;
-    T* dOb = dO64 + hf * QT * DS;
-    const float* lse_b = lse64 + hf * QT;
-    const float* dl_b = dl64 + hf * QT;
-    if (qbase + QT > k0) {
-    float pt[2][4], dst[2][4];
-    __builtin_amdgcn_s_setprio(1);
-    const int krow = k0 + lo;
-#pragma unroll
-    for (int nt = 0; nt < 2; ++nt) {
-      floatx4 st = (floatx4)(0.f);
-      floatx4 dpt = (floatx4)(0.f);
+    for (int hf = 0; hf < QTT / QT; ++hf) {
+      const int qbase = qt * QTT + hf * QT;
+      if (qbase + QT <= k0) continue;
+      const T* Qb = Q_lds + cur * QTT * DS + hf * QT * DS;
+      const T* dOb = dO_lds + cur * QTT * DS + hf * QT * DS;
+      const float* lse_b = lse_lds + cur * QTT + hf * QT;
+      const float* dl_b = dl_lds + cur * QTT + hf * QT;
+
+      floatx16 sc, dp;
+#pragma unroll
+      for (int g = 0; g < 4; ++g) {
+        const floatx4 l4 = *(const floatx4*)(lse_b + 8 * g + 4 * hi5);
+        const floatx4 d4 = *(const floatx4*)(dl_b + 8 * g + 4 * hi5);
+#pragma unroll
+        for (int i = 0; i < 4; ++i) { sc[4 * g + i] = l4[i]; dp[4 * g + i] = d4[i]; }
+      }
+      __builtin_amdgcn_s_setprio(1);
 #pragma unroll
       for (int kc = 0; kc < NKC; ++kc) {
-        frag qa = *(const frag*)(Qb + (nt * 16 + lo) * DS + kc * 32 + hi * 8);
-        st = MF::mma(qa, k_frag[kc], st);
-        frag doa = *(const frag*)(dOb + (nt * 16 + lo) * DS + kc * 32 + hi * 8);
-        dpt = MF::mma(doa, v_frag[kc], dpt);
-      }
-      const floatx4 lse4 = *(const floatx4*)(lse_b + nt * 16 + hi * 4);
-      const floatx4 dl4 = *(const floatx4*)(dl_b + nt * 16 + hi * 4);
-#pragma unroll
-      for (int r = 0; r < 4; ++r) {
-        const int qrow = qbase + nt * 16 + hi * 4 + r;
-        float pv = 0.f;
-        if (krow <= qrow && krow < S && qrow < S)
-          pv = __expf(st[r] * scale - lse4[r]);
-        pt[nt][r] = pv;
-        dst[nt][r] = pv * (dpt[r] - dl4[r]) * scale;
-      }
-    }
-
-    T* Pw = PT_lds + wave * 16 * QS;
-    using P4 = typename Pack4<DT>::V;
-#pragma unroll
-    for (int nt = 0; nt < 2; ++nt) {
-      P4 pk;
-#pragma unroll
-      for (int r = 0; r < 4; ++r) ((T*)&pk)[r] = TR::fromF(pt[nt][r]);
-      *(P4*)(Pw + lo * QS + nt * 16 + hi * 4) = pk;
-    }
-    frag pa = *(const frag*)(Pw + lo * QS + hi * 8);
-#pragma unroll
-    for (int dn = 0; dn < NDN; ++dn) {
-      frag bd = trread_bfrag<DT>(dOb, 0, dn * 16, DS, lane);
-      dv_acc[dn] = MF::mma(pa, bd, dv_acc[dn]);
-    }
-
-    T* Dw = DS_lds + wave * 16 * QS;
-#pragma unroll
-    for (int nt = 0; nt < 2; ++nt) {
-      P4 dk4;
-#pragma unroll
-      for (int r = 0; r < 4; ++r) ((T*)&dk4)[r] = TR::fromF(dst[nt][r]);
-      *(P4*)(Dw + lo * QS + nt * 16 + hi * 4) = dk4;
-    }
-    frag da = *(const frag*)(Dw + lo * QS + hi * 8);
-#pragma unroll
-    for (int dn = 0; dn < NDN; ++dn) {
-      frag bq = trread_bfrag<DT>(Qb, 0, dn * 16, DS, lane);
-      dk_acc[dn] = MF::mma(da, bq, dk_acc[dn]);
-    }
-    __builtin_amdgcn_s_setprio(0);
-    }
+        frag qa = *(const frag*)(Qb + lo32 * DS + kc * 16 + hi5 * 8);
+        sc = MF::mma(qa, k_frag[kc], sc);
+        frag doa = *(const frag*)(dOb + lo32 * DS + kc * 16 + hi5 * 8);
+        dp = MF::mma(doa, v_frag[kc], dp);
+      }
+      __builtin_amdgcn_s_setprio(0);
+
+#pragma unroll
+      for (int r = 0; r < 16; ++r) sc[r] = exp2_fast(sc[r] * c2);
+      if (qbase < k0 + QT || qbase + QT > S) {
+#pragma unroll
+        for (int r = 0; r < 16; ++r) {
+          const int qr = qbase + (r & 3) + 8 * (r >> 2) + 4 * hi5;
+          if (key > qr || qr >= S) sc[r] = 0.f;
+        }
+      }
+#pragma unroll
+      for (int r = 0; r < 16; ++r) dp[r] *= sc[r];
+      frag pf[2], dsf[2];
+#pragma unroll
+      for (int c = 0; c < 2; ++c) {
+        pf[c] = pack_frag32<DT>(sc, c);
+        dsf[c] = pack_frag32<DT>(dp, c);
+      }
+
+      __builtin_amdgcn_s_setprio(1);
+#pragma unroll
+      for (int mt = 0; mt < NMT; ++mt)
+#pragma unroll
+        for (int c = 0; c < 2; ++c) {
+          frag da = trread_afrag32<DT>(dOb, c * 16, mt * 32, DS, lane);
+          dv_acc[mt] = MF::mma(da, pf[c], dv_acc[mt]);
+          frag qa = trread_afrag32<DT>(Qb, c * 16, mt * 32, DS, lane);
+          dk_acc[mt] = MF::mma(qa, dsf[c], dk_acc[mt]);
+        }
+      __builtin_amdgcn_s_setprio(0);
     }
 
     if (qt + 1 < nQT2) write_qtile(cur ^ 1);
     __syncthreads();
   }
 
-  const int64_t dvoff = dv_sb ? ((int64_t)b * dv_sb + (int64_t)h * dv_sh) : qoff;
-  const int64_t dv_rs = dv_sb ? dv_sr : (int64_t)D;
-#pragma unroll
-  for (int r = 0; r < 4; ++r) {
-    const int krow = k0 + hi * 4 + r;
-    if (krow >= S) continue;
-#pragma unroll
-    for (int dn = 0; dn < NDN; ++dn) {
-      dk_out[qoff + (int64_t)krow * D + dn * 16 + lo] = TR::fromF(dk_acc[dn][r]);
-      dv_out[dvoff + (int64_t)krow * dv_rs + dn * 16 + lo] = TR::fromF(dv_acc[dn][r]);
-    }
-  }
-}
-
-template <int DT, int D>
-__global__ __launch_bounds__(512) void attn_bwd_dq_kernel(
-    typename DTraits<DT>::T* __restrict__ dq_out,
-    const typename DTraits<DT>::T* __restrict__ do_,
-    const typename DTraits<DT>::T* __restrict__ q,
-    const typename DTraits<DT>::T* __restrict__ k,
-    const typename DTraits<DT>::T* __restrict__ v,
-    const float* __restrict__ lse, const float* __restrict__ delta,
-    int B, int Hq, int Hkv, int S, float scale,
-    int64_t g_sb, int64_t g_sh, int64_t g_sr,
-    int64_t v_sb, int64_t v_sh, int64_t v_sr) {
-  using TR = DTraits<DT>;
-  using T = typename TR::T;
-  using MF = MFMA16<DT>;
-  using frag = typename MF::frag;
-  constexpr int KT = 64;
-  constexpr int KS = KT + 8;
-  constexpr int DS = D + 8;
-  constexpr int NKC = D / 32;
-  constexpr int NDN = D / 16;
-
-  extern __shared__ __attribute__((aligned(16))) char smem_raw[];
-  T* K_lds = (T*)smem_raw;
-  T* V_lds = K_lds + 3 * KT * DS;
-  T* S_lds = V_lds + 3 * KT * DS;
-
-  const int lane = threadIdx.x & 63;
-  const int wave = threadIdx.x >> 6;
-  const int lo = lane & 15;
-  const int hi = lane >> 4;
-
-  const int nQT = (S + 127) / 128;
-  int bid = blockIdx.x;
-  const int qt = bid % nQT;
-  const int h = (bid / nQT) % Hq;
-  const int b = bid / (nQT * Hq);
-  const int hkv = h / (Hq / Hkv);
-
-  const int q0 = qt * 128 + wave * 16;
-  const int64_t qoff = (((int64_t)b * Hq + h) * S) * D;
-  const int64_t kvoff = (((int64_t)b * Hkv + hkv) * S) * D;
-  const int64_t lseoff = ((int64_t)b * Hq + h) * S;
-  const int64_t voff = v_sb ? ((int64_t)b * v_sb + (int64_t)hkv * v_sh) : kvoff;
-  const int64_t v_rs = v_sb ? v_sr : (int64_t)D;
-
-  frag q_frag[NKC], do_frag[NKC];
-  float lse_q, dl_q;
-  const int qrow_l = q0 + lo;
-  {
-    const int qr_c = qrow_l < S ? qrow_l : S - 1;
-    const int64_t gbase = (int64_t)b * g_sb + (int64_t)h * g_sh;
-#pragma unroll
-    for (int kc = 0; kc < NKC; ++kc) {
-      q_frag[kc] = *(const frag*)(q + qoff + (int64_t)qr_c * D + kc * 32 + hi * 8);
-      do_frag[kc] = *(const frag*)(do_ + gbase + (int64_t)qr_c * g_sr + kc * 32 + hi * 8);
-    }
-    lse_q = lse[lseoff + qr_c];
-    dl_q = delta[lseoff + qr_c];
-  }
-
-  floatx4 dq_acc[NDN];
-#pragma unroll
-  for (int dn = 0; dn < NDN; ++dn) dq_acc[dn] = (floatx4)(0.f);
-
-  const int kv_end = min(S, qt * 128 + 128);
-  const int n_kt = (kv_end + KT - 1) / KT;
-
-  const int st_t = (int)threadIdx.x;
-  const bool st_on = st_t < (KT * D) / 8;
-  const int st_row = st_t / (D / 8);
-  const int st_c8 = (st_t % (D / 8)) * 8;
-  frag kregA, vregA, kregB, vregB;
-
-  auto load_ktile = [&](int kt, frag& kr, frag& vr) {
-    if (st_on) {
-      const int krow = kt * KT + st_row;
-      const int kr_c = krow < S ? krow : S - 1;
-      kr = *(const frag*)(k + kvoff + (int64_t)kr_c * D + st_c8);
-      vr = *(const frag*)(v + voff + (int64_t)kr_c * v_rs + st_c8);
-    }
-  };
-  auto write_ktile = [&](int buf, const frag& kr, const frag& vr) {
-    if (st_on) {
-      *(frag*)(K_lds + buf * KT * DS + st_row * DS + st_c8) = kr;
-      *(frag*)(V_lds + buf * KT * DS + st_row * DS + st_c8) = vr;
-    }
-  };
-
-  load_ktile(0, kregA, vregA);
-  write_ktile(0, kregA, vregA);
-  if (1 < n_kt) load_ktile(1, kregB, vregB);
-  __syncthreads();
-
-  for (int kt = 0; kt < n_kt; ++kt) {
-    const int kbase = kt * KT;
-    const int cur = kt % 3;
-    T* Kb = K_lds + cur * KT * DS;
-    T* Vb = V_lds + cur * KT * DS;
-    if (kt + 2 < n_kt) {
-      if ((kt + 2) & 1) load_ktile(kt + 2, kregB, vregB);
-      else load_ktile(kt + 2, kregA, vregA);
-    }
-
-    if (kbase < q0 + 16) {
-    float ds[4][4];
-    __builtin_amdgcn_s_setprio(1);
-#pragma unroll
-    for (int nt = 0; nt < 4; ++nt) {
-      floatx4 st = (floatx4)(0.f), dpt = (floatx4)(0.f);
-#pragma unroll
-      for (int kc = 0; kc < NKC; ++kc) {
-        frag ka = *(const frag*)(Kb + (nt * 16 + lo) * DS + kc * 32 + hi * 8);
-        st = MF::mma(ka, q_frag[kc], st);
-        frag va = *(const frag*)(Vb + (nt * 16 + lo) * DS + kc * 32 + hi * 8);
-        dpt = MF::mma(va, do_frag[kc], dpt);
-      }
-#pragma unroll
-      for (int r = 0; r < 4; ++r) {
-        const int kcol = kbase + nt * 16 + hi * 4 + r;
-        float pv = 0.f;
-        if (kcol <= qrow_l && kcol < S && qrow_l < S)
-          pv = __expf(st[r] * scale - lse_q);
-        ds[nt][r] = pv * (dpt[r] - dl_q) * scale;
-      }
-    }
-
-    T* Sw = S_lds + wave * 16 * KS;
-    using P4 = typename Pack4<DT>::V;
-#pragma unroll
-    for (int nt = 0; nt < 4; ++nt) {
-      P4 s4;
-#pragma unroll
-      for (int r = 0; r < 4; ++r) ((T*)&s4)[r] = TR::fromF(ds[nt][r]);
-      *(P4*)(Sw + lo * KS + nt * 16 + hi * 4) = s4;
-    }
-    frag da[2];
-#pragma unroll
-    for (int c = 0; c < 2; ++c) da[c] = *(const frag*)(Sw + lo * KS + c * 32 + hi * 8);
-#pragma unroll
-    for (int dn = 0; dn < NDN; ++dn)
-#pragma unroll
-      for (int c = 0; c < 2; ++c) {
-        frag bk = trread_bfrag<DT>(Kb, c * 32, dn * 16, DS, lane);
-        dq_acc[dn] = MF::mma(da[c], bk, dq_acc[dn]);
-      }
-    __builtin_amdgcn_s_setprio(0);
-    }
-
-    if (kt + 1 < n_kt) {
-      if ((kt + 1) & 1) write_ktile((kt + 1) % 3, kregB, vregB);
-      else write_ktile((kt + 1) % 3, kregA, vregA);
-    }
-    __syncthreads();
-  }
-
-#pragma unroll
-  for (int r = 0; r < 4; ++r) {
-    const int qrow = q0 + hi * 4 + r;
-    if (qrow >= S) continue;
-#pragma unroll
-    for (int dn = 0; dn < NDN; ++dn)
-      dq_out[qoff + (int64_t)qrow * D + dn * 16 + lo] = TR::fromF(dq_acc[dn][r]);
-  }
-}
-
-
-template <int DT, int D>
-__global__ __launch_bounds__(256) void attn_bwd_dkdv_v3_kernel(
-    typename DTraits<DT>::T* __restrict__ dk_out,
-    typename DTraits<DT>::T* __restrict__ dv_out,
-    const typename DTraits<DT>::T* __restrict__ do_,
-    const typename DTraits<DT>::T* __restrict__ q,
-    const typename DTraits<DT>::T* __restrict__ k,
-    const typename DTraits<DT>::T* __restrict__ v,
-    const float* __restrict__ lse, const float* __restrict__ delta,
-    int B, int Hq, int Hkv, int S, float scale,
-    int64_t g_sb, int64_t g_sh, int64_t g_sr) {
-  using TR = DTraits<DT>;
-  using T = typename TR::T;
-  using MF = MFMA32<DT>;
-  using frag = typename MF::frag;
-  constexpr int QT = 32;
-  constexpr int QS = QT + 8;
-  constexpr int DS = D + 8;
-  constexpr int NKC = D / 16;
-  constexpr int NMT = D / 32;
-
-  extern __shared__ __attribute__((aligned(16))) char smem_raw[];
-  T* Q_lds = (T*)smem_raw;
-  T* dO_lds = Q_lds + 2 * QT * DS;
-  T* PT_lds = dO_lds + 2 * QT * DS;
-  T* DST_lds = PT_lds + 4 * 32 * QS;
-  float* lse_lds = (float*)(DST_lds + 4 * 32 * QS);
-  float* dl_lds = lse_lds + 2 * QT;
-
-  const int lane = threadIdx.x & 63;
-  const int wave = threadIdx.x >> 6;
-  const int lo32 = lane & 31;
-  const int hi5 = lane >> 5;
-
-  const int nKT = (S + 127) / 128;
-  int bid = blockIdx.x;
-  const int kt = bid % nKT;
-  const int h = (bid / nKT) % Hq;
-  const int b = bid / (nKT * Hq);
-  const int hkv = h / (Hq / Hkv);
-
-  const int k0 = kt * 128 + wave * 32;
-  const int64_t qoff = (((int64_t)b * Hq + h) * S) * D;
-  const int64_t kvoff = (((int64_t)b * Hkv + hkv) * S) * D;
-  const int64_t lseoff = ((int64_t)b * Hq + h) * S;
-
-  const int kr_c0 = (k0 + lo32) < S ? (k0 + lo32) : S - 1;
-  const T* kbase_p = k + kvoff + (int64_t)kr_c0 * D + hi5 * 8;
-  const T* vbase_p = v + kvoff + (int64_t)kr_c0 * D + hi5 * 8;
-
-  floatx16 dv_acc[NMT], dk_acc[NMT];
-#pragma unroll
-  for (int mt = 0; mt < NMT; ++mt) { dv_acc[mt] = (floatx16)(0.f); dk_acc[mt] = (floatx16)(0.f); }
-
-  const int qstart = (kt * 128) / QT;
-  const int nQT2 = (S + QT - 1) / QT;
-
-  const int st_t = (int)threadIdx.x;
-  const bool st_on = st_t < (QT * D) / 8;
-  const int st_row = st_t / (D / 8);
-  const int st_c8 = (st_t % (D / 8)) * 8;
-  shortx8 qreg, dreg;
-  float lse_reg = 0.f, dl_reg = 0.f;
-  const int64_t gbase = (int64_t)b * g_sb + (int64_t)h * g_sh;
-
-  auto load_qtile = [&](int qt2) {
-    const int qrow = qt2 * QT + st_row;
-    const int qr_c = qrow < S ? qrow : S - 1;
-    if (st_on) {
-      qreg = *(const shortx8*)(q + qoff + (int64_t)qr_c * D + st_c8);
-      dreg = *(const shortx8*)(do_ + gbase + (int64_t)qr_c * g_sr + st_c8);
-    }
-    if (st_t < QT) {
-      const int rr = qt2 * QT + st_t;
-      const int rr_c = rr < S ? rr : S - 1;
-      lse_reg = lse[lseoff + rr_c];
-      dl_reg = delta[lseoff + rr_c];
-    }
-  };
-  auto write_qtile = [&](int buf) {
-    if (st_on) {
-      *(shortx8*)(Q_lds + buf * QT * DS + st_row * DS + st_c8) = qreg;
-      *(shortx8*)(dO_lds + buf * QT * DS + st_row * DS + st_c8) = dreg;
-    }
-    if (st_t < QT) {
-      lse_lds[buf * QT + st_t] = lse_reg;
-      dl_lds[buf * QT + st_t] = dl_reg;
-    }
-  };
-
-  load_qtile(qstart);
-  write_qtile(0);
-  __syncthreads();
-
-  for (int qt2 = qstart; qt2 < nQT2; ++qt2) {
-    const int qbase = qt2 * QT;
-    const int cur = (qt2 - qstart) & 1;
-    T* Qb = Q_lds + cur * QT * DS;
-    T* dOb = dO_lds + cur * QT * DS;
-    const float* lse_b = lse_lds + cur * QT;
-    const float* dl_b = dl_lds + cur * QT;
-    if (qt2 + 1 < nQT2) load_qtile(qt2 + 1);
-
-    floatx16 st = (floatx16)(0.f), dpt = (floatx16)(0.f);
-    __builtin_amdgcn_s_setprio(1);
-#pragma unroll
-    for (int kc = 0; kc < NKC; ++kc) {
-      frag ka = *(const frag*)(kbase_p + kc * 16);
-      frag bq = *(const frag*)(Qb + lo32 * DS + kc * 16 + hi5 * 8);
-      st = MF::mma(ka, bq, st);
-      frag va = *(const frag*)(vbase_p + kc * 16);
-      frag bd = *(const frag*)(dOb + lo32 * DS + kc * 16 + hi5 * 8);
-      dpt = MF::mma(va, bd, dpt);
-    }
-    __builtin_amdgcn_s_setprio(0);
-
-    const int qcol = qbase + lo32;
-    const float lse_q = lse_b[lo32];
-    const float dl_q = dl_b[lo32];
-    const bool full = (qbase >= k0 + 32) && (qbase + QT <= S);
-    float pt[16], dst[16];
-#pragma unroll
-    for (int r = 0; r < 16; ++r) {
-      float pv;
-      if (full) {
-        pv = __expf(st[r] * scale - lse_q);
-      } else {
-        const int krow = k0 + (r & 3) + 8 * (r >> 2) + 4 * hi5;
-        pv = 0.f;
-        if (krow <= qcol && krow < S && qcol < S)
-          pv = __expf(st[r] * scale - lse_q);
-      }
-      pt[r] = pv;
-      dst[r] = pv * (dpt[r] - dl_q) * scale;
-    }
-
-    T* Pw = PT_lds + wave * 32 * QS;
-#pragma unroll
-    for (int r = 0; r < 16; ++r)
-      Pw[((r & 3) + 8 * (r >> 2) + 4 * hi5) * QS + lo32] = TR::fromF(pt[r]);
-    frag pa[2];
-#pragma unroll
-    for (int c = 0; c < 2; ++c)
-      pa[c] = *(const frag*)(Pw + lo32 * QS + c * 16 + hi5 * 8);
-    __builtin_amdgcn_s_setprio(1);
+  if (key < S) {
+    const int64_t dvoff = dv_sb ? ((int64_t)b * dv_sb + (int64_t)h * dv_sh) : qoff;
+    const int64_t dv_rs = dv_sb ? dv_sr : (int64_t)D;
+    T* dkp = dk_out + qoff + (int64_t)key * D;
+    T* dvp = dv_out + dvoff + (int64_t)key * dv_rs;
 #pragma unroll
     for (int mt = 0; mt < NMT; ++mt)
 #pragma unroll
-      for (int c = 0; c < 2; ++c) {
-        frag bd = trread_afrag32<DT>(dOb, c * 16, mt * 32, DS, lane);
-        dv_acc[mt] = MF::mma(pa[c], bd, dv_acc[mt]);
-      }
-    __builtin_amdgcn_s_setprio(0);
-
-    T* Dw = DST_lds + wave * 32 * QS;
-#pragma unroll
-    for (int r = 0; r < 16; ++r)
-      Dw[((r & 3) + 8 * (r >> 2) + 4 * hi5) * QS + lo32] = TR::fromF(dst[r]);
-    frag da[2];
-#pragma unroll
-    for (int c = 0; c < 2; ++c)
-      da[c] = *(const frag*)(Dw + lo32 * QS + c * 16 + hi5 * 8);
-    __builtin_amdgcn_s_setprio(1);
-#pragma unroll
-    for (int mt = 0; mt < NMT; ++mt)
-#pragma unroll
-      for (int c = 0; c < 2; ++c) {
-        frag bq = trread_afrag32<DT>(Qb, c * 16, mt * 32, DS, lane);
-        dk_acc[mt] = MF::mma(da[c], bq, dk_acc[mt]);
-      }
-    __builtin_amdgcn_s_setprio(0);
-
-    if (qt2 + 1 < nQT2) write_qtile(cur ^ 1);
-    __syncthreads();
-  }
-
-#pragma unroll
-  for (int r = 0; r < 16; ++r) {
-    const int krow = k0 + (r & 3) + 8 * (r >> 2) + 4 * hi5;
-    if (krow >= S) continue;
-#pragma unroll
-    for (int mt = 0; mt < NMT; ++mt) {
-      dk_out[qoff + (int64_t)krow * D + mt * 32 + lo32] = TR::fromF(dk_acc[mt][r]);
-      dv_out[qoff + (int64_t)krow * D + mt * 32 + lo32] = TR::fromF(dv_acc[mt][r]);
-    }
-  }
-}
-
-template <int DT, int D, int WANT_DK>
-__global__ __launch_bounds__(256) void attn_bwd_split32_kernel(
-    typename DTraits<DT>::T* __restrict__ out,
-    const typename DTraits<DT>::T* __restrict__ do_,
-    const typename DTraits<DT>::T* __restrict__ q,
-    const typename DTraits<DT>::T* __restrict__ k,
-    const typename DTraits<DT>::T* __restrict__ v,
-    const float* __restrict__ lse, const float* __restrict__ delta,
-    int B, int Hq, int Hkv, int S, float scale,
-    int64_t g_sb, int64_t g_sh, int64_t g_sr,
-    int64_t v_sb, int64_t v_sh, int64_t v_sr,
-    int64_t o_sb, int64_t o_sh, int64_t o_sr) {
-  using TR = DTraits<DT>;
-  using T = typename TR::T;
-  using MF = MFMA32<DT>;
-  using frag = typename MF::frag;
-  using P4 = typename Pack4<DT>::V;
-  constexpr int QT = 32;
-  constexpr int QS = QT + 8;
-  constexpr int DS = D + 8;
-  constexpr int NKC = D / 16;
-  constexpr int NMT = D / 32;
-
-  extern __shared__ __attribute__((aligned(16))) char smem_raw[];
-  T* Q_lds = (T*)smem_raw;
-  T* dO_lds = Q_lds + 2 * QT * DS;
-  T* PT_lds = dO_lds + 2 * QT * DS;
-  float* lse_lds = (float*)(PT_lds + 4 * 32 * QS);
-  float* dl_lds = lse_lds + 2 * QT;
-
-  const int lane = threadIdx.x & 63;
-  const int wave = threadIdx.x >> 6;
-  const int lo32 = lane & 31;
-  const int hi5 = lane >> 5;
-
-  const int nKT = (S + 127) / 128;
-  int bid = blockIdx.x;
-  const int kt = bid % nKT;
-  const int h = (bid / nKT) % Hq;
-  const int b = bid / (nKT * Hq);
-  const int hkv = h / (Hq / Hkv);
-
-  const int k0 = kt * 128 + wave * 32;
-  const int64_t qoff = (((int64_t)b * Hq + h) * S) * D;
-  const int64_t kvoff = (((int64_t)b * Hkv + hkv) * S) * D;
-  const int64_t lseoff = ((int64_t)b * Hq + h) * S;
-  const int64_t voff = v_sb ? ((int64_t)b * v_sb + (int64_t)hkv * v_sh) : kvoff;
-  const int64_t v_rs = v_sb ? v_sr : (int64_t)D;
-
-  const int kr_c0 = (k0 + lo32) < S ? (k0 + lo32) : S - 1;
-  const T* kbase_p = k + kvoff + (int64_t)kr_c0 * D + hi5 * 8;
-  const T* vbase_p = v + voff + (int64_t)kr_c0 * v_rs + hi5 * 8;
-
-  floatx16 acc[NMT];
-#pragma unroll
-  for (int mt = 0; mt < NMT; ++mt) acc[mt] = (floatx16)(0.f);
-
-  const int qstart = (kt * 128) / QT;
-  const int nQT2 = (S + QT - 1) / QT;
-
-  const int st_t = (int)threadIdx.x;
-  const bool st_on = st_t < (QT * D) / 8;
-  const int st_row = st_t / (D / 8);
-  const int st_c8 = (st_t % (D / 8)) * 8;
-  shortx8 qreg, dreg;
-  float lse_reg = 0.f, dl_reg = 0.f;
-  const int64_t gbase = (int64_t)b * g_sb + (int64_t)h * g_sh;
-
-  auto load_qtile = [&](int qt2) {
-    const int qrow = qt2 * QT + st_row;
-    const int qr_c = qrow < S ? qrow : S - 1;
-    if (st_on) {
-      qreg = *(const shortx8*)(q + qoff + (int64_t)qr_c * D + st_c8);
-      dreg = *(const shortx8*)(do_ + gbase + (int64_t)qr_c * g_sr + st_c8);
-    }
-    if (st_t < QT) {
-      const int rr = qt2 * QT + st_t;
-      const int rr_c = rr < S ? rr : S - 1;
-      lse_reg = lse[lseoff + rr_c];
-      if (WANT_DK) dl_reg = delta[lseoff + rr_c];
-    }
-  };
-  auto write_qtile = [&](int buf) {
-    if (st_on) {
-      *(shortx8*)(Q_lds + buf * QT * DS + st_row * DS + st_c8) = qreg;
-      *(shortx8*)(dO_lds + buf * QT * DS + st_row * DS + st_c8) = dreg;
-    }
-    if (st_t < QT) {
-      lse_lds[buf * QT + st_t] = lse_reg;
-      if (WANT_DK) dl_lds[buf * QT + st_t] = dl_reg;
-    }
-  };
-
-  load_qtile(qstart);
-  write_qtile(0);
-  __syncthreads();
-
-  for (int qt2 = qstart; qt2 < nQT2; ++qt2) {
-    const int qbase = qt2 * QT;
-    const int cur = (qt2 - qstart) & 1;
-    T* Qb = Q_lds + cur * QT * DS;
-    T* dOb = dO_lds + cur * QT * DS;
-    const float* lse_b = lse_lds + cur * QT;
-    const float* dl_b = dl_lds + cur * QT;
-    if (qt2 + 1 < nQT2) load_qtile(qt2 + 1);
-
-    floatx16 st = (floatx16)(0.f), dpt = (floatx16)(0.f);
-    __builtin_amdgcn_s_setprio(1);
-#pragma unroll
-    for (int kc = 0; kc < NKC; ++kc) {
-      frag qa = *(const frag*)(Qb + lo32 * DS + kc * 16 + hi5 * 8);
-      frag kb = *(const frag*)(kbase_p + kc * 16);
-      st = MF::mma(qa, kb, st);
-      if (WANT_DK) {
-        frag doa = *(const frag*)(dOb + lo32 * DS + kc * 16 + hi5 * 8);
-        frag vb = *(const frag*)(vbase_p + kc * 16);
-        dpt = MF::mma(doa, vb, dpt);
-      }
-    }
-    __builtin_amdgcn_s_setprio(0);
-
-    const int krow = k0 + lo32;
-    const bool full = (qbase >= k0 + 32) && (qbase + QT <= S);
-    T* Pw = PT_lds + wave * 32 * QS;
-#pragma unroll
-    for (int g = 0; g < 4; ++g) {
-      const int qloc = 8 * g + 4 * hi5;
-      const floatx4 lse4 = *(const floatx4*)(lse_b + qloc);
-      floatx4 dl4;
-      if (WANT_DK) dl4 = *(const floatx4*)(dl_b + qloc);
-      P4 pk;
-#pragma unroll
-      for (int r = 0; r < 4; ++r) {
-        const int i = g * 4 + r;
-        float pv;
-        if (full) {
-          pv = __expf(st[i] * scale - lse4[r]);
-        } else {
-          const int qrow = qbase + qloc + r;
-          pv = 0.f;
-          if (krow <= qrow && krow < S && qrow < S)
-            pv = __expf(st[i] * scale - lse4[r]);
-        }
-        if (WANT_DK) pv = pv * (dpt[i] - dl4[r]) * scale;
-        ((T*)&pk)[r] = TR::fromF(pv);
-      }
-      *(P4*)(Pw + lo32 * QS + qloc) = pk;
-    }
-
-    frag pa[2];
-#pragma unroll
-    for (int c = 0; c < 2; ++c)
-      pa[c] = *(const frag*)(Pw + lo32 * QS + c * 16 + hi5 * 8);
-    __builtin_amdgcn_s_setprio(1);
-#pragma unroll
-    for (int mt = 0; mt < NMT; ++mt)
-#pragma unroll
-      for (int c = 0; c < 2; ++c) {
-        frag bb = trread_afrag32<DT>(WANT_DK ? Qb : dOb, c * 16, mt * 32, DS, lane);
-        acc[mt] = MF::mma(pa[c], bb, acc[mt]);
-      }
-    __builtin_amdgcn_s_setprio(0);
-
-    if (qt2 + 1 < nQT2) write_qtile(cur ^ 1);
-    __syncthreads();
-  }
-
-  const int64_t obase = o_sb ? ((int64_t)b * o_sb + (int64_t)h * o_sh) : qoff;
-  const int64_t o_rs = o_sb ? o_sr : (int64_t)D;
-#pragma unroll
-  for (int r = 0; r < 16; ++r) {
-    const int kr = k0 + (r & 3) + 8 * (r >> 2) + 4 * hi5;
-    if (kr >= S) continue;
-#pragma unroll
-    for (int mt = 0; mt < NMT; ++mt)
-      out[obase + (int64_t)kr * o_rs + mt * 32 + lo32] = TR::fromF(acc[mt][r]);
-  }
-}
-
-template <int DT, int D>
-__global__ __launch_bounds__(256) void attn_bwd_dq_v3_kernel(
-    typename DTraits<DT>::T* __restrict__ dq_out,
-    const typename DTraits<DT>::T* __restrict__ do_,
-    const typename DTraits<DT>::T* __restrict__ q,
-    const typename DTraits<DT>::T* __restrict__ k,
-    const typename DTraits<DT>::T* __restrict__ v,
-    const float* __restrict__ lse, const float* __restrict__ delta,
-    int B, int Hq, int Hkv, int S, float scale,
-    int64_t g_sb, int64_t g_sh, int64_t g_sr) {
-  using TR = DTraits<DT>;
-  using T = typename TR::T;
-  using MF = MFMA32<DT>;
-  using frag = typename MF::frag;
-  constexpr int KT = 32;
-  constexpr int KS = KT + 8;
-  constexpr int DS = D + 8;
-  constexpr int NKC = D / 16;
-  constexpr int NMT = D / 32;
-
-  extern __shared__ __attribute__((aligned(16))) char smem_raw[];
-  T* K_lds = (T*)smem_raw;
-  T* V_lds = K_lds + 2 * KT * DS;
-  T* S_lds = V_lds + 2 * KT * DS;
-
-  const int lane = threadIdx.x & 63;
-  const int wave = threadIdx.x >> 6;
-  const int lo32 = lane & 31;
-  const int hi5 = lane >> 5;
-
-  const int nQT = (S + 127) / 128;
-  int bid = blockIdx.x;
-  const int qt = bid % nQT;
-  const int h = (bid / nQT) % Hq;
-  const int b = bid / (nQT * Hq);
-  const int hkv = h / (Hq / Hkv);
-
-  const int q0 = qt * 128 + wave * 32;
-  const int64_t qoff = (((int64_t)b * Hq + h) * S) * D;
-  const int64_t kvoff = (((int64_t)b * Hkv + hkv) * S) * D;
-  const int64_t lseoff = ((int64_t)b * Hq + h) * S;
-
-  frag q_frag[NKC], do_frag[NKC];
-  float lse_r[16], dl_r[16];
-  {
-    const int qrow = q0 + lo32;
-    const int qr_c = qrow < S ? qrow : S - 1;
-    const int64_t gb = (int64_t)b * g_sb + (int64_t)h * g_sh;
-#pragma unroll
-    for (int kc = 0; kc < NKC; ++kc) {
-      q_frag[kc] = *(const frag*)(q + qoff + (int64_t)qr_c * D + kc * 16 + hi5 * 8);
-      do_frag[kc] = *(const frag*)(do_ + gb + (int64_t)qr_c * g_sr + kc * 16 + hi5 * 8);
-    }
-#pragma unroll
-    for (int r = 0; r < 16; ++r) {
-      const int rr = q0 + (r & 3) + 8 * (r >> 2) + 4 * hi5;
-      const int rr_c = rr < S ? rr : S - 1;
-      lse_r[r] = lse[lseoff + rr_c];
-      dl_r[r] = delta[lseoff + rr_c];
-    }
-  }
-
-  floatx16 dq_acc[NMT];
-#pragma unroll
-  for (int mt = 0; mt < NMT; ++mt) dq_acc[mt] = (floatx16)(0.f);
-
-  const int kv_end = min(S, qt * 128 + 128);
-  const int n_kt = (kv_end + KT - 1) / KT;
-
-  const int st_t = (int)threadIdx.x;
-  const bool st_on = st_t < (KT * D) / 8;
-  const int st_row = st_t / (D / 8);
-  const int st_c8 = (st_t % (D / 8)) * 8;
-  shortx8 kreg, vreg;
-
-  auto load_ktile = [&](int kt2) {
-    if (st_on) {
-      const int krow = kt2 * KT + st_row;
-      const int kr_c = krow < S ? krow : S - 1;
-      kreg = *(const shortx8*)(k + kvoff + (int64_t)kr_c * D + st_c8);
-      vreg = *(const shortx8*)(v + kvoff + (int64_t)kr_c * D + st_c8);
-    }
-  };
-  auto write_ktile = [&](int buf) {
-    if (st_on) {
-      *(shortx8*)(K_lds + buf * KT * DS + st_row * DS + st_c8) = kreg;
-      *(shortx8*)(V_lds + buf * KT * DS + st_row * DS + st_c8) = vreg;
-    }
-  };
-
-  load_ktile(0);
-  write_ktile(0);
-  __syncthreads();
-
-  for (int kt2 = 0; kt2 < n_kt; ++kt2) {
-    const int kbase = kt2 * KT;
-    const int cur = kt2 & 1;
-    T* Kb = K_lds + cur * KT * DS;
-    T* Vb = V_lds + cur * KT * DS;
-    if (kt2 + 1 < n_kt) load_ktile(kt2 + 1);
-
-    floatx16 st = (floatx16)(0.f), dpt = (floatx16)(0.f);
-    __builtin_amdgcn_s_setprio(1);
-#pragma unroll
-    for (int kc = 0; kc < NKC; ++kc) {
-      frag bk = *(const frag*)(Kb + lo32 * DS + kc * 16 + hi5 * 8);
-      st = MF::mma(q_frag[kc], bk, st);
-      frag bv = *(const frag*)(Vb + lo32 * DS + kc * 16 + hi5 * 8);
-      dpt = MF::mma(do_frag[kc], bv, dpt);
-    }
-    __builtin_amdgcn_s_setprio(0);
-
-    const int kcol = kbase + lo32;
-    const bool full = (kbase + KT <= q0) && (kbase + KT <= S) && (q0 + 32 <= S);
-    float ds[16];
-#pragma unroll
-    for (int r = 0; r < 16; ++r) {
-      float pv;
-      if (full) {
-        pv = __expf(st[r] * scale - lse_r[r]);
-      } else {
-        const int qrow = q0 + (r & 3) + 8 * (r >> 2) + 4 * hi5;
-        pv = 0.f;
-        if (kcol <= qrow && kcol < S && qrow < S)
-          pv = __expf(st[r] * scale - lse_r[r]);
-      }
-      ds[r] = pv * (dpt[r] - dl_r[r]) * scale;
-    }
-
-    T* Sw = S_lds + wave * 32 * KS;
-#pragma unroll
-    for (int r = 0; r < 16; ++r)
-      Sw[((r & 3) + 8 * (r >> 2) + 4 * hi5) * KS + lo32] = TR::fromF(ds[r]);
-    frag da[2];
-#pragma unroll
-    for (int c = 0; c < 2; ++c)
-      da[c] = *(const frag*)(Sw + lo32 * KS + c * 16 + hi5 * 8);
-    __builtin_amdgcn_s_setprio(1);
-#pragma unroll
-    for (int mt = 0; mt < NMT; ++mt)
-#pragma unroll
-      for (int c = 0; c < 2; ++c) {
-        frag bk = trread_afrag32<DT>(Kb, c * 16, mt * 32, DS, lane);
-        dq_acc[mt] = MF::mma(da[c], bk, dq_acc[mt]);
-      }
-    __builtin_amdgcn_s_setprio(0);
-
-    if (kt2 + 1 < n_kt) write_ktile(cur ^ 1);
-    __syncthreads();
-  }
-
-#pragma unroll
-  for (int r = 0; r < 16; ++r) {
-    const int qrow = q0 + (r & 3) + 8 * (r >> 2) + 4 * hi5;
-    if (qrow >= S) continue;
-#pragma unroll
-    for (int mt = 0; mt < NMT; ++mt)
-      dq_out[qoff + (int64_t)qrow * D + mt * 32 + lo32] = TR::fromF(dq_acc[mt][r]);
+      for (int g = 0; g < 4; ++g) {
+        store4<DT>(dkp + mt * 32 + 8 * g + 4 * hi5, dk_acc[mt], g, scale);
+        store4<DT>(dvp + mt * 32 + 8 * g + 4 * hi5, dv_acc[mt], g, 1.f);
+      }
   }
 }
 
@@ -1409,24 +885,6 @@
   static int cached = -1;
   if (cached < 0) {
     const char* e = getenv("DK_ATTN_V2");
-    cached = (e && e[0] == '1') ? 1 : 0;
-  }
-  return cached == 1;
-}
-
-static bool use_bwd_split32() {
-  static int v = -1;
-  if (v < 0) {
-    const char* e = getenv("DK_ATTN_BWD_SPLIT32");
-    v = (e && e[0] == '1') ? 1 : 0;
-  }
-  return v != 0;
-}
-
-static bool use_bwd_v3() {
-  static int cached = -1;
-  if (cached < 0) {
-    const char* e = getenv("DK_ATTN_BWD_V3");
     cached = (e && e[0] == '1') ? 1 : 0;
   }
   return cached == 1;
@@ -1511,42 +969,12 @@
                                 int64_t dv_sb, int64_t dv_sh, int64_t dv_sr,
                                 dkStream stream) {
   using T = typename DTraits<DT>::T;
-  constexpr int QT = 32, QS = QT + 8, DS = D + 8;
-  if (use_bwd_split32()) {
-    const int nKTs = (int)((S + 127) / 128);
-    const int grids = (int)(B * Hq * nKTs);
-    const size_t ldss = sizeof(T) * (4 * QT * DS + 4 * 32 * QS) + sizeof(float) * 4 * QT;
-    hipLaunchKernelGGL((attn_bwd_split32_kernel<DT, D, 0>), dim3(grids), dim3(256), ldss,
-                       (hipStream_t)stream, (T*)dv_o, (const T*)do_, (const T*)q,
-                       (const T*)k, (const T*)v, lse, delta, (int)B, (int)Hq,
-                       (int)Hkv, (int)S, scale, g_sb, g_sh, g_sr, v_sb, v_sh, v_sr,
-                       dv_sb, dv_sh, dv_sr);
-    DK_CHECK_LAUNCH();
-    hipLaunchKernelGGL((attn_bwd_split32_kernel<DT, D, 1>), dim3(grids), dim3(256), ldss,
-                       (hipStream_t)stream, (T*)dk_o, (const T*)do_, (const T*)q,
-                       (const T*)k, (const T*)v, lse, delta, (int)B, (int)Hq,
-                       (int)Hkv, (int)S, scale, g_sb, g_sh, g_sr, v_sb, v_sh, v_sr,
-                       0, 0, 0);
-    DK_CHECK_LAUNCH();
-    return 0;
-  }
-  if (use_bwd_v3() && v_sb == 0 && dv_sb == 0) {
-    const int nKT3 = (int)((S + 127) / 128);
-    const int grid3 = (int)(B * Hq * nKT3);
-    const size_t lds3 = sizeof(T) * (4 * QT * DS + 2 * 4 * 32 * QS)
-                        + sizeof(float) * 4 * QT;
-    hipLaunchKernelGGL((attn_bwd_dkdv_v3_kernel<DT, D>), dim3(grid3), dim3(256), lds3,
-                       (hipStream_t)stream, (T*)dk_o, (T*)dv_o, (const T*)do_,
-                       (const T*)q, (const T*)k, (const T*)v, lse, delta,
-                       (int)B, (int)Hq, (int)Hkv, (int)S, scale, g_sb, g_sh, g_sr);
-    DK_CHECK_LAUNCH();
-    return 0;
-  }
+  constexpr int QTT = 32, DS = D + 8;
+  if (((uintptr_t)dv_o & 7) || (dv_sb | dv_sh | dv_sr) & 3) return (int)hipErrorInvalidValue;
   const int nKT = (int)((S + 127) / 128);
   const int grid = (int)(B * Hq * nKT);
-  constexpr int QTT = 64;
-  const size_t lds = sizeof(T) * (4 * QTT * DS + 2 * 8 * 16 * QS) + sizeof(float) * 4 * QTT;
-  hipLaunchKernelGGL((attn_bwd_dkdv_kernel<DT, D>), dim3(grid), dim3(512), lds,
+  const size_t lds = sizeof(T) * (4 * QTT * DS) + sizeof(float) * 4 * QTT;
+  hipLaunchKernelGGL((attn_bwd_dkdv_kernel<DT, D>), dim3(grid), dim3(256), lds,
                      (hipStream_t)stream, (T*)dk_o, (T*)dv_o, (const T*)do_,
                      (const T*)q, (const T*)k, (const T*)v, lse, delta,
                      (int)B, (int)Hq, (int)Hkv, (int)S, scale, g_sb, g_sh, g_sr,
@@ -1583,23 +1011,11 @@
                               int64_t v_sb, int64_t v_sh, int64_t v_sr,
                               dkStream stream) {
   using T = typename DTraits<DT>::T;
-  constexpr int KT = 32, KS = KT + 8, DS = D + 8;
-  constexpr int KT2 = 64, KS2 = KT2 + 8;
-  if (use_bwd_v3() && v_sb == 0) {
-    const int nQT3 = (int)((S + 127) / 128);
-    const int grid3 = (int)(B * Hq * nQT3);
-    const size_t lds3 = sizeof(T) * (4 * KT * DS + 4 * 32 * KS);
-    hipLaunchKernelGGL((attn_bwd_dq_v3_kernel<DT, D>), dim3(grid3), dim3(256), lds3,
-                       (hipStream_t)stream, (T*)dq_o, (const T*)do_, (const T*)q,
-                       (const T*)k, (const T*)v, lse, delta, (int)B, (int)Hq,
-                       (int)Hkv, (int)S, scale, g_sb, g_sh, g_sr);
-    DK_CHECK_LAUNCH();
-    return 0;
-  }
+  constexpr int KT = 64, DS = D + 8;
   const int nQT = (int)((S + 127) / 128);
   const int grid = (int)(B * Hq * nQT);
-  const size_t lds = sizeof(T) * (6 * KT2 * DS + 8 * 16 * KS2);
-  hipLaunchKernelGGL((attn_bwd_dq_kernel<DT, D>), dim3(grid), dim3(512), lds,
+  const size_t lds = sizeof(T) * (4 * KT * DS);
+  hipLaunchKernelGGL((attn_bwd_dq_kernel<DT, D>), dim3(grid), dim3(256), lds,
                      (hipStream_t)stream, (T*)dq_o, (const T*)do_, (const T*)q,
                      (const T*)k, (const T*)v, lse, delta, (int)B, (int)Hq,
                      (int)Hkv, (int)S, scale, g_sb, g_sh, g_sr, v_sb, v_sh, v_sr);
```

New measurement: 644,700 tokens/s (median of 6 runs). +5.5%, better.
